# DarioSamo/sm64rt-legacy-renderer

Hardware: AMD Instinct MI355X
Metric: Mrays/s (primary+shadow), sample scene 1080p 1spp (higher is better)
Workload: dtype f32

## Files before the change

### sm64rt-legacy-renderer_amd/csrc/pass_common.h

```cpp
#pragma once
#include <type_traits>
#include "kernels.h"
#include "shade.h"

struct Pixel { uint32_t x, y; bool valid; };

enum TileShape { TILE_SQUARE = 0, TILE_ROWS = 1 };
template <int SHAPE> struct TileDim { static constexpr int W = SHAPE == TILE_SQUARE ? 16 : 32, H = SHAPE == TILE_SQUARE ? 16 : 8; };

DEV uint32_t owned_strips(PRef P) {
    const uint32_t all = (uint32_t)(P.tileY1 - P.tileY0 + 15) / 16;
    return all > (uint32_t)P.stripRank ? (all - (uint32_t)P.stripRank + (uint32_t)P.stripCount - 1) / (uint32_t)P.stripCount : 0u;
}
template <int SHAPE = TILE_SQUARE> DEV uint32_t tile_count(PRef P) {
    return (uint32_t)((P.width + TileDim<SHAPE>::W - 1) / TileDim<SHAPE>::W) * owned_strips(P) * (16u / TileDim<SHAPE>::H);
}
template <int SHAPE = TILE_SQUARE> DEV Pixel tile_pixel_at(PRef P, uint32_t tile, uint32_t wave, uint32_t lane) {
    constexpr uint32_t TW = TileDim<SHAPE>::W, TH = TileDim<SHAPE>::H, perStrip = 16u / TH;
    const uint32_t tilesX = ((uint32_t)P.width + TW - 1) / TW;
    const uint32_t tx = tile % tilesX, lt = tile / tilesX;
    const uint32_t strip = (lt / perStrip) * (uint32_t)P.stripCount + (uint32_t)P.stripRank;
    Pixel p;
    if (SHAPE == TILE_SQUARE) { p.x = tx * TW + (wave & 1) * 8 + (lane & 7); p.y = (wave >> 1) * 8 + (lane >> 3); }
    else { p.x = tx * TW + (lane & 31); p.y = wave * 2 + (lane >> 5); }
    p.y += (uint32_t)P.tileY0 + strip * 16 + (lt % perStrip) * TH;
    p.valid = p.x < (uint32_t)P.width && p.y < (uint32_t)P.tileY1;
    return p;
}
template <int SHAPE = TILE_SQUARE> DEV Pixel tile_pixel(PRef P, uint32_t tile) {
    return tile_pixel_at<SHAPE>(P, tile, threadIdx.x >> 6, threadIdx.x & 63);
}

DEV bool row_owned(PRef P, int y) { return (((y - P.tileY0) / 16) % P.stripCount) == P.stripRank; }

constexpr uint32_t stack_words(bool cached) { return cached ? RT_STACK_LDS_CACHED / 2 : RT_STACK_LDS; }
DEV TraceStack make_stack(PRef P, uint32_t *ldsStack, uint32_t wordsPerLane) {
    TraceStack s;
    uint32_t *block = ldsStack + (threadIdx.x >> 6) * wordsPerLane * RT_LANES;
    s.lds = (LdsU32Ptr)(block + (threadIdx.x & 63u));
    s.lds16 = (LdsI16Ptr)block + (threadIdx.x & 63u);
    s.spill = (GlobalU32Ptr)(P.traversalStack + ((size_t)blockIdx.x * blockDim.x + threadIdx.x) * (RT_STACK_SPILL_HEADER + RT_STACK_SPILL) + RT_STACK_SPILL_HEADER);
    s.cache = nullptr; s.ldsEntries = RT_STACK_LDS;
    return s;
}
DEV void light_columns(ShadeEnv &env, float *intensities, uint8_t *indices, uint32_t slots) {
    const uint32_t at = (threadIdx.x >> 6) * slots * RT_LANES + (threadIdx.x & 63u);
    env.lightIntensity = intensities + at; env.lightIndex = indices + at;
}

DEV uint32_t light_slots(PRef P) { return (P.lightCount < RT64_MAX_LIGHTS ? P.lightCount : (uint32_t)RT64_MAX_LIGHTS) + 1u; }


template <bool CACHED> DEV void traversal_env(PRef P, ShadeEnv &env, uint32_t *ldsStack, const u32x4_lds *dynLds) {
    env.stk = make_stack(P, ldsStack, stack_words(CACHED)); env.cnt = TraceCounts(); env.shadowRays = 0;
    env.lightIntensity = nullptr; env.lightIndex = nullptr;
    if (CACHED) env.stk.use_cache(dynLds);
}
template <bool CACHED, bool STATIC_COLUMNS = true, int BLOCK = RT_BLOCK>
DEV void shading_env(PRef P, ShadeEnv &env, uint32_t *ldsStack, float *ldsLightIntensity, uint8_t *ldsLightIndex, u32x4_lds *dynLds) {
    env.stk = make_stack(P, ldsStack, stack_words(CACHED)); env.cnt = TraceCounts(); env.shadowRays = 0;
    if (STATIC_COLUMNS) light_columns(env, ldsLightIntensity, ldsLightIndex, RT64_MAX_LIGHTS + 1);
    if (STATIC_COLUMNS && !CACHED) return;
    if (CACHED) { fill_scene_cache(P, dynLds); env.stk.use_cache(dynLds); }
    float *li = reinterpret_cast<float *>(dynLds + (CACHED ? P.cacheWords : 0u));
    light_columns(env, li, reinterpret_cast<uint8_t *>(li + light_slots(P) * (CACHED ? blockDim.x : (uint32_t)BLOCK)), light_slots(P));
}

DEV void flush_env(PRef P, const ShadeEnv &env, int pass, int rayCounter, uint32_t rays) {
    flush_counts(P, env.cnt, pass);
    if (!P.countTraversal) return;
    unsigned long long a = rays, b = env.shadowRays;
#pragma unroll
    for (int d = 32; d >= 1; d >>= 1) { a += __shfl_down(a, d, 64); b += __shfl_down(b, d, 64); }
    if ((threadIdx.x & 63) == 0) { unsigned long long *ctr = P.counters + (size_t)(blockIdx.x % RT_COUNTER_STRIPES) * CTR_COUNT; if (a) atomicAdd(&ctr[rayCounter], a); if (b) atomicAdd(&ctr[CTR_SHADOW], b); }
}

struct SurfaceHit { float key, t, u, v; uint32_t instance, prim; bool hit; };

template <bool KLIST, bool CACHED = false>
DEV uint32_t trace_surface(PRef P, ShadeEnv &env, IRef I, size_t pixel, f3 o, f3 d, const RayDiff &rayDiff,
                           uint32_t px, uint32_t py, SurfaceHit &best) {
    float oo[3] = { o.x, o.y, o.z }, dd[3] = { d.x, d.y, d.z };
    best.hit = false; best.key = INFINITY;
    uint32_t nhits = 0;
    const size_t stride = (size_t)P.width * (size_t)P.height;
    trace_ray<CACHED>(P, oo, dd, RT_RAY_MIN_DISTANCE, RT_RAY_MAX_DISTANCE, true, env.stk,
              [&](float t, float u, float v, uint32_t instance, uint32_t prim, float &tmax, uint32_t instFlags, float instDepthBias) -> bool {
                  const GpuInstance &in = P.instances[instance];
                  const float key = t - instDepthBias;
                  if (!KLIST) {
                      if (key < best.key) { best.key = key; best.t = t; best.u = u; best.v = v; best.instance = instance; best.prim = prim; best.hit = true; }
                  }
                  else {
                      if (in.cc.optTextureEdge) {
                          HitRecord tmp;
                          if (!surface_anyhit(P, instance, prim, t, u, v, d, rayDiff, px, py, tmp)) return false;
                      }
                      uint32_t hi = nhits < RT64_MAX_HIT_QUERIES ? nhits : RT64_MAX_HIT_QUERIES;
                      while (hi > 0) {
                          const uint4 prev = I.klistA[(size_t)(hi - 1) * stride + pixel];
                          if (!(key < __uint_as_float(prev.x))) break;
                          I.klistA[(size_t)hi * stride + pixel] = prev;
                          I.klistB[(size_t)hi * stride + pixel] = I.klistB[(size_t)(hi - 1) * stride + pixel];
                          hi--;
                      }
                      if (hi < RT64_MAX_HIT_QUERIES) {
                          I.klistA[(size_t)hi * stride + pixel] = make_uint4(__float_as_uint(key), __float_as_uint(u), __float_as_uint(v), prim);
                          I.klistB[(size_t)hi * stride + pixel] = make_uint2(__float_as_uint(t), instance);
                          ++nhits;
                          if (hi == RT64_MAX_HIT_QUERIES - 1 && t < tmax) tmax = t;
                      }
                      if (!(instFlags & GPU_INST_OPAQUE)) return false;
                  }
                  const float lim = key + P.maxDepthBias;
                  if (lim < tmax) tmax = lim;
                  return false;
              }, env.cnt);
    return KLIST ? nhits : (best.hit ? 1u : 0u);
}

constexpr int TRACE_WAVES = 4;
static unsigned rt_grid(const FrameParams &P) {
    const unsigned tiles = owned_tiles(P, true);
    return tiles < 1u ? 1u : (tiles < (unsigned)RT_GRID_BLOCKS ? tiles : (unsigned)RT_GRID_BLOCKS);
}
static size_t cached_lds_bytes(const FrameParams &P, bool lights) {
    const size_t slots = (P.lightCount < RT64_MAX_LIGHTS ? P.lightCount : (uint32_t)RT64_MAX_LIGHTS) + 1u;
    return (size_t)P.cacheWords * 16 + (lights ? (slots * RT_BLOCK * 5 + 15) / 16 * 16 : 0);
}
static inline dim3 image_grid(int w, int rows) { return dim3((unsigned)(w + 31) / 32, (unsigned)(rows + 7) / 8); }
template <class... Params, class... Args>
static inline void enqueue(void (*kernel)(Params...), dim3 grid, unsigned block, size_t ldsBytes, hipStream_t s, const Args &... args) {
    hipLaunchKernelGGL(kernel, grid, dim3(block), ldsBytes, s, args...);
}
template <class... Params, class... Args>
static inline hipError_t launch(void (*kernel)(Params...), dim3 grid, unsigned block, size_t ldsBytes, hipStream_t s, const Args &... args) {
    enqueue(kernel, grid, block, ldsBytes, s, args...);
    return hipGetLastError();
}
template <class F> static inline auto with_flag(bool flag, F &&f) { return flag ? f(std::true_type()) : f(std::false_type()); }
```

### sm64rt-legacy-renderer_amd/csrc/passes.hip

```cpp
#include "pass_common.h"
#include "raster_pixel.h"

#ifdef RT_ASSUME_SIMPLE
#define RT_LAUNCHER(name) name##_simple
#define RT_ROUTE_SIMPLE(call)
#else
#define RT_LAUNCHER(name) name
#define RT_ROUTE_SIMPLE(call) if (P.simpleKernels) return call
#endif

namespace {

DEV void klist_slot(PRef P, IRef I, size_t pixel, uint32_t hit, uint4 &a, uint2 &b) {
    const size_t stride = (size_t)P.width * (size_t)P.height;
    a = I.klistA[(size_t)hit * stride + pixel];
    b = I.klistB[(size_t)hit * stride + pixel];
}
template <bool KLIST>
DEV bool surface_entry(PRef P, IRef I, size_t pixel, uint32_t hit, const SurfaceHit &best, SurfaceHit &e) {
    if (!KLIST) { e = best; return true; }
    if (hit > RT64_MAX_HIT_QUERIES) return false;
    uint4 a; uint2 b; klist_slot(P, I, pixel, hit, a, b);
    e.instance = b.y; e.prim = a.w; e.t = __uint_as_float(b.x); e.u = __uint_as_float(a.y); e.v = __uint_as_float(a.z); e.hit = true; e.key = __uint_as_float(a.x);
    return true;
// ... 198 lines not shown
        f3 indirect = mk3(q_f16(P.ambientBaseColor[0] + P.ambientNoGIColor[0]), q_f16(P.ambientBaseColor[1] + P.ambientNoGIColor[1]), q_f16(P.ambientBaseColor[2] + P.ambientNoGIColor[2]));
        result = diffuse * (directStored + indirect);
        result = lerp3(diffuse, result, d.w);
    }
    else result = xyz(d);
    return result;
}
DEV void compose_lean_pixel(PRef P, IRef I, size_t i, f3 directStored) {
    f4 d = load_rgba8(I.diffuse, i);
    f3 result;
    if (d.w > RT_EPSILON) {
        f3 diffuse = xyz(d);
        f3 indirect = mk3(q_f16(P.ambientBaseColor[0] + P.ambientNoGIColor[0]), q_f16(P.ambientBaseColor[1] + P.ambientNoGIColor[1]), q_f16(P.ambientBaseColor[2] + P.ambientNoGIColor[2]));
        result = diffuse * (directStored + indirect);
        result = lerp3(diffuse, result, d.w);
    }
    else result = xyz(d);
    reinterpret_cast<float4 *>(I.output)[i] = make_float4(result.x, result.y, result.z, 1.0f);
    if (!P.separatePost) store_rgba8(I.final, i, result.x, result.y, result.z, 1.0f);
}

template <bool CACHED>
DEV f3 direct_light_pixel(PRef P, ShadeEnv &env, uint32_t px, uint32_t py, f3 rayDirection, int instanceId, f3 position, f3 normal, f3 specular) {
    f3 selfLight; float specularExponent;
    waterfall((uint32_t)instanceId, [&](uint32_t k) { const RT64_MATERIAL mk = load_const(&P.instances[k].material); selfLight = ld_v3(mk.selfLight); specularExponent = mk.specularExponent; });
    f3 resDirect = compute_lights_random<CACHED>(P, env, px, py, rayDirection, (uint32_t)instanceId, position, normal, specular, P.maxLights, true);
    resDirect = resDirect + selfLight;
    float eyeLambert = fmaxf(dot3(normal, -rayDirection), 0.0f);
    f3 eyeReflected = reflect3(rayDirection, normal);
    float eyeSpec = s_pow(fmaxf(saturatef(dot3(eyeReflected, -rayDirection)), 0.0f), specularExponent);
    f3 eyeD = mk3(P.eyeLightDiffuseColor[0], P.eyeLightDiffuseColor[1], P.eyeLightDiffuseColor[2]), eyeS = mk3(P.eyeLightSpecularColor[0], P.eyeLightSpecularColor[1], P.eyeLightSpecularColor[2]);
    return resDirect + (eyeD * eyeLambert + eyeS * (specular * eyeSpec));
}

template <bool FULL, bool CACHED = false>
__global__ __launch_bounds__(RT_BLOCK, DIRECT_WAVES) void direct_kernel(FrameParams Pv, ViewImages Iv, int cur) {
    PRef P = *kernel_params(); IRef I = *kernel_images(); (void)Pv; (void)Iv; (void)I;
    __shared__ uint32_t ldsStack[stack_words(CACHED) * RT_BLOCK];
    __shared__ float ldsLightIntensity[CACHED ? 1 : (RT64_MAX_LIGHTS + 1) * RT_BLOCK];
    __shared__ uint8_t ldsLightIndex[CACHED ? 1 : (RT64_MAX_LIGHTS + 1) * RT_BLOCK];
    extern __shared__ u32x4_lds dynLds[];
    ShadeEnv env; shading_env<CACHED>(P, env, ldsStack, ldsLightIntensity, ldsLightIndex, dynLds);
    const uint32_t tiles = tile_count<DIRECT_TILE>(P);
    for (uint32_t tile = blockIdx.x; tile < tiles; tile += gridDim.x) {
        PRef P = *kernel_params_here(); IRef I = *kernel_images_here();
        Pixel p = tile_pixel<DIRECT_TILE>(P, tile);
        if (!p.valid) continue;
        const uint32_t px = p.x, py = p.y;
        const size_t i = (size_t)py * (size_t)P.width + px;
        const int instanceId = I.instanceId[i];
        if (instanceId < 0) {
            store_rgba16f(I.directLight[cur], i, 1.0f, 1.0f, 1.0f, 0.0f);
            if (FULL) store_rgba16f(I.filteredDirect[1], i, 1.0f, 1.0f, 1.0f, 0.0f);
            else compose_lean_pixel(P, I, i, mk3s(1.0f));
            continue;
        }
        f3 o, rayDirection; f2 ndc;
        primary_ray(P, px, py, o, rayDirection, ndc);
        const float4 pos4 = reinterpret_cast<const float4 *>(I.shadingPosition)[i];
        f3 position = mk3(pos4.x, pos4.y, pos4.z), normal = xyz(load_rgba16f(I.shadingNormal, i)), specular = xyz(load_rgba16f(I.shadingSpecular, i));
        f3 newDirect = mk3s(0.0f); float historyLength = 0.0f;
        if (P.diReproject) {
            long j; float w = history_weight(P, I, i, px, py, normal, cur, j);
            f4 prevAccum = j >= 0 ? load_rgba16f(I.directLight[cur ^ 1], (size_t)j) : mk4(0, 0, 0, 0);
            newDirect = xyz(prevAccum); historyLength = prevAccum.w * w;
        }
        const f3 resDirect = direct_light_pixel<CACHED>(P, env, px, py, rayDirection, instanceId, position, normal, specular);
        historyLength = fminf(historyLength + 1.0f, 64.0f);
        newDirect = lerp3(newDirect, resDirect, s_rcp(historyLength));
        store_rgba16f(I.directLight[cur], i, newDirect.x, newDirect.y, newDirect.z, historyLength);
        if (FULL) store_rgba16f(I.filteredDirect[1], i, newDirect.x, newDirect.y, newDirect.z, historyLength);
        else compose_lean_pixel(P, I, i, mk3(q_f16(newDirect.x), q_f16(newDirect.y), q_f16(newDirect.z)));
    }
    flush_env(P, env, PASS_DIRECT, CTR_PRIMARY, 0);
}

constexpr int LEAN_WAVES = 3;
DEV bool wave_tile_of(uint32_t seq, uint32_t tiles, uint32_t &tileSeq, uint32_t &quadrant) {
    const uint32_t xcd = seq & 7u, j = seq >> 3;
    quadrant = j & 3u; tileSeq = (j >> 2) * 8u + xcd;
    return tileSeq < tiles;
}
template <bool CACHED, bool FULL, int WAVES, int BLOCK = RT_BLOCK>
__global__ __launch_bounds__(BLOCK, WAVES) void lean_frame_kernel(FrameParams Pv, ViewImages Iv, int32_t *hitInstance, int cur, int ownedY0, int ownedY1) {
    PRef P = *kernel_params(); IRef I = *kernel_images(); (void)Pv; (void)Iv; (void)I;
    __shared__ uint32_t ldsStack[stack_words(CACHED) * BLOCK];
    extern __shared__ u32x4_lds dynLds[];
    ShadeEnv env; shading_env<CACHED, false, BLOCK>(P, env, ldsStack, nullptr, nullptr, dynLds);
    uint32_t rays = 0;
    TraceCounts primaryCnt = TraceCounts();
    const uint32_t tiles = tile_count(P);
    const uint32_t trips = BLOCK == RT_BLOCK ? tiles : ((tiles + 7u) / 8u) * 32u;
    if (P.tileTiming && (threadIdx.x & 63u) == 0u) {
        uint32_t hwId; asm volatile("s_getreg_b32 %0, hwreg(HW_REG_HW_ID)" : "=s"(hwId));
        P.tileTiming[2 * ((size_t)blockIdx.x * (BLOCK / 64) + (threadIdx.x >> 6))] = make_uint4((uint32_t)__builtin_amdgcn_s_memrealtime(), (uint32_t)__builtin_amdgcn_s_memtime(), hwId, 1u);
    }
    __shared__ uint32_t ldsTripCost;
    uint32_t tileOfTrip = 0xFFFFFFFFu, visitsBefore = 0;
    const bool costed = BLOCK != RT_BLOCK && P.tileCost != nullptr;
    if (costed && threadIdx.x == 0) ldsTripCost = 0;
    auto note_cost = [&]() { if (costed) atomicMax(&ldsTripCost, env.cnt.nodes + env.cnt.tris - visitsBefore); };
    auto flush_cost = [&](PRef P) {
        if (!costed || tileOfTrip == 0xFFFFFFFFu) return;
        __syncthreads();
        if (threadIdx.x == 0) { atomicMax(&P.tileCost[tileOfTrip], ldsTripCost); ldsTripCost = 0; }
        tileOfTrip = 0xFFFFFFFFu;
    };
    for (uint32_t trip = blockIdx.x; trip < trips; trip += gridDim.x) {
        PRef P = *kernel_params_here(); IRef I = *kernel_images_here();
        Pixel p;
        if (BLOCK == RT_BLOCK) p = tile_pixel(P, tiles - 1u - trip);
        else {
            uint32_t tileSlot, quadrant;
            flush_cost(P);
            if (!wave_tile_of(trip, tiles, tileSlot, quadrant)) continue;
            tileOfTrip = P.tileOrder ? P.tileOrder[tileSlot] : tileSlot;
            p = tile_pixel_at(P, tiles - 1u - tileOfTrip, quadrant, threadIdx.x & 63u);
            visitsBefore = env.cnt.nodes + env.cnt.tris;
        }
        if (!p.valid) continue;
        const uint32_t px = p.x, py = p.y;
        const size_t i = (size_t)py * (size_t)P.width + px;
        f3 o, rayDirection; f2 ndc;
        primary_ray(P, px, py, o, rayDirection, ndc);
        RayDiff noDiff; noDiff.dOdx = noDiff.dOdy = noDiff.dDdx = noDiff.dDdy = mk3s(0.0f);
        SurfaceHit h;
        const TraceCounts before = env.cnt;
        const uint32_t nhits = trace_surface<false, CACHED>(P, env, I, i, o, rayDirection, noDiff, px, py, h);
        primaryCnt.nodes += env.cnt.nodes - before.nodes; primaryCnt.tris += env.cnt.tris - before.tris;
        rays++;
        const bool keepRecords = FULL || hitInstance != nullptr;
        if (keepRecords) {
            uint4 rec;
            if (h.hit) { rec.x = __float_as_uint(h.t); rec.y = __float_as_uint(h.u); rec.z = __float_as_uint(h.v); rec.w = h.prim; hitInstance[i] = (int32_t)h.instance; }
            else { rec.x = rec.y = rec.z = rec.w = 0xFFFFFFFFu; hitInstance[i] = -1; }
            reinterpret_cast<uint4 *>(I.primaryHit)[i] = rec;
        }

        PrimaryResolve R;
        resolve_primary<false, false, FULL>(P, I, env, px, py, i, o, rayDirection, ndc, h, nhits, R);
        if (FULL) {
            store_primary<true>(P, I, i, cur, rayDirection, R);
            if ((int)py < ownedY0 || (int)py >= ownedY1) { note_cost(); continue; }
        }
        const f4 diffuse = mk4(q_unorm8(R.color.x), q_unorm8(R.color.y), q_unorm8(R.color.z), q_unorm8(R.color.w));
        f3 direct = mk3s(1.0f); float historyLength = 0.0f;
        if (R.instanceId >= 0) {
            const f3 normal = mk3(q_f16(R.normal.x), q_f16(R.normal.y), q_f16(R.normal.z));
            const f3 specular = mk3(q_f16(R.specular.x), q_f16(R.specular.y), q_f16(R.specular.z));
            const f3 resDirect = direct_light_pixel<CACHED>(P, env, px, py, rayDirection, R.instanceId, R.position, normal, specular);
            historyLength = 1.0f;
            direct = lerp3(mk3s(0.0f), resDirect, s_rcp(historyLength));
        }
        if (keepRecords) store_rgba16f(I.directLight[cur], i, direct.x, direct.y, direct.z, historyLength);
        if (FULL) { store_rgba16f(I.filteredDirect[1], i, direct.x, direct.y, direct.z, historyLength); note_cost(); continue; }
        const f3 result = compose_lean_value(P, diffuse, mk3(q_f16(direct.x), q_f16(direct.y), q_f16(direct.z)));
        if (P.separatePost) reinterpret_cast<float4 *>(I.output)[i] = make_float4(result.x, result.y, result.z, 1.0f);
        else {
            uint32_t bits = (uint32_t)to_unorm8(result.x) | ((uint32_t)to_unorm8(result.y) << 8) | ((uint32_t)to_unorm8(result.z) << 16) | ((uint32_t)to_unorm8(1.0f) << 24);
            if (P.rasterFgCount) {
                const int wx0 = __builtin_amdgcn_readfirstlane((int)(px & ~7u)), wy0 = __builtin_amdgcn_readfirstlane((int)(py & ~7u));
                bool loaded = true, dirty = false;
                raster_blend_pixel(P.rasterFg, static_cast<const RasterTri *>(P.rasterFgTris), P.rasterFgCount, P.textures, (int)px, (int)py, true, wx0, wx0 + 7, wy0, wy0 + 7, nullptr, bits, loaded, dirty);
            }
            reinterpret_cast<uint32_t *>(I.final)[i] = bits;
            if (P.finalPacked) {
                const uint32_t rel = py - (uint32_t)P.tileY0, prow = ((rel >> 4) / (uint32_t)P.stripCount) * 16u + (rel & 15u);
                P.finalPacked[(size_t)prow * (size_t)P.width + px] = bits;
            }
        }
        note_cost();
    }
    flush_cost(P);
    if (P.tileTiming) {
        uint32_t worst = env.cnt.nodes + env.cnt.tris, total = worst;
#pragma unroll
        for (int d = 32; d >= 1; d >>= 1) { worst = max(worst, (uint32_t)__shfl_xor((int)worst, d, 64)); total += (uint32_t)__shfl_xor((int)total, d, 64); }
        if ((threadIdx.x & 63u) == 0u)
            P.tileTiming[2 * ((size_t)blockIdx.x * (BLOCK / 64) + (threadIdx.x >> 6)) + 1] = make_uint4((uint32_t)__builtin_amdgcn_s_memrealtime(), (uint32_t)__builtin_amdgcn_s_memtime(), worst, (total << 8) | 1u);
    }
    TraceCounts directCnt = TraceCounts(); directCnt.nodes = env.cnt.nodes - primaryCnt.nodes; directCnt.tris = env.cnt.tris - primaryCnt.tris;
    flush_counts(P, primaryCnt, PASS_PRIMARY_TRACE);
    env.cnt = directCnt;
    flush_env(P, env, PASS_DIRECT, CTR_PRIMARY, rays);
}


template <bool KLIST, bool CACHED>
DEV f3 second_bounce_radiance(PRef P, ShadeEnv &env, IRef I, size_t i, uint32_t px, uint32_t py, f3 rayOrigin, f3 normal, uint32_t noiseFrame, f3 ambientBase, f3 ambient) {
    const f3 rayDirection = cos_hemisphere_blue_noise(P, px, py, noiseFrame, normal);
    RayDiff rd; rd.dOdx = rd.dOdy = rd.dDdx = rd.dDdy = mk3s(0.0f);
    SurfaceHit best;
    const uint32_t nhits = trace_surface<KLIST, CACHED>(P, env, I, i, rayOrigin, rayDirection, rd, px, py, best);
    f3 resPosition = mk3s(0.0f), resNormal = mk3s(0.0f), resSpecular = mk3s(0.0f); f4 resColor = mk4(0, 0, 0, 1); int resInstanceId = -1;
    for (uint32_t hit = 0; hit < nhits; hit++) {
        HitRecord r;
        if (!surface_record<KLIST>(P, I, i, hit, best, rayDirection, rd, px, py, r)) continue;
        f4 hitColor = r.color;
        float alphaContrib = resColor.w * hitColor.w;
        if (alphaContrib >= RT_EPSILON) {
            const RT64_MATERIAL &m = P.instances[r.instanceId].material;
            resPosition = rayOrigin + rayDirection * (r.dist + m.depthBias);
            resNormal = r.normal; resSpecular = ld_v3(m.specularColor) * r.specular;
            resColor.x += hitColor.x * alphaContrib; resColor.y += hitColor.y * alphaContrib; resColor.z += hitColor.z * alphaContrib;
            resColor.w *= (1.0f - hitColor.w);
            resInstanceId = (int)r.instanceId;
        }
        if (resColor.w <= RT_EPSILON) break;
    }
    f3 resIndirect = ambientBase;
    if (resInstanceId >= 0) {
// ... 610 lines not shown
        const f3 bgColor = sky_over_background_envmap(P, rayDirection);
        RayDiff rd; rd.dOdx = rd.dOdy = rd.dDdx = rd.dDdy = mk3s(0.0f);
        SurfaceHit best;
        const uint32_t nhits = trace_surface<KLIST, CACHED>(P, env, I, i, shadingPosition, rayDirection, rd, px, py, best);
        rays++;
        const RT64_MATERIAL &pm = P.instances[instanceId].material;
        f3 resPosition = mk3s(0.0f), resNormal = mk3s(0.0f), resSpecular = mk3s(0.0f), resTransparent = mk3s(0.0f); f4 resColor = mk4(0, 0, 0, 1); int resInstanceId = -1;
        for (uint32_t hit = 0; hit < nhits; hit++) {
            HitRecord r;
            if (!surface_record<KLIST>(P, I, i, hit, best, rayDirection, rd, px, py, r)) continue;
            f4 hitColor = r.color;
            float alphaContrib = resColor.w * hitColor.w;
            if (alphaContrib >= RT_EPSILON) {
                const RT64_MATERIAL &m = P.instances[r.instanceId].material;
                bool usesLighting = m.lightGroupMaskBits > 0;
                f3 vertexPosition = shadingPosition + rayDirection * (r.dist + m.depthBias);
                if (m.fogEnabled) {
                    f4 fog = fog_from_origin(m, vertexPosition, shadingPosition);
                    resTransparent = resTransparent + xyz(fog) * (fog.w * alphaContrib);
                    alphaContrib *= (1.0f - fog.w);
                }
                f3 vertexNormal = r.normal;
                f3 specular = ld_v3(m.specularColor) * r.specular;
                if (m.reflectionFactor > RT_EPSILON) {
                    float fresnelAmount = fresnel_reflect_amount(vertexNormal, rayDirection, m.reflectionFactor, pm.reflectionFresnelFactor);
                    newReflectionAlpha += fresnelAmount * alphaContrib * reflectionAlpha;
                }
                if (usesLighting) { resColor.x += hitColor.x * alphaContrib; resColor.y += hitColor.y * alphaContrib; resColor.z += hitColor.z * alphaContrib; }
                else resTransparent = resTransparent + (xyz(hitColor) * alphaContrib) * (ambient + ld_v3(m.selfLight));
                resPosition = vertexPosition; resNormal = vertexNormal; resSpecular = specular; resInstanceId = (int)r.instanceId;
                resColor.w *= (1.0f - hitColor.w);
            }
            if (resColor.w <= RT_EPSILON) break;
        }
        f3 rgb = xyz(resColor);
        if (resInstanceId >= 0) {
            f3 directLight = compute_lights_random<CACHED>(P, env, px, py, rayDirection, (uint32_t)resInstanceId, resPosition, resNormal, resSpecular, 1, false) + ld_v3(P.instances[resInstanceId].material.selfLight);
            rgb = rgb * (ambient + directLight);
            I.reflState0[i] = make_uint4(__float_as_uint(resPosition.x), __float_as_uint(resPosition.y), __float_as_uint(resPosition.z), (uint32_t)resInstanceId);
            I.reflState1[i] = make_uint4(pack_rgba16f_lo(rayDirection.x, rayDirection.y), pack_rgba16f_lo(rayDirection.z, 0.0f), pack_rgba16f_lo(resNormal.x, resNormal.y), pack_rgba16f_lo(resNormal.z, 0.0f));
            I.reflTag[i] = frameTag;
        }
        rgb = rgb + (bgColor * resColor.w + resTransparent);
        const f3 HighlightColor = mk3(1.0f, 1.05f, 1.2f), ShadowColor = mk3(0.1f, 0.05f, 0.0f);
        float shine = pm.reflectionShineFactor;
        rgb = lerp3(rgb, HighlightColor, s_pow(fmaxf(rayDirection.y, 0.0f) * shine, 3.0f));
        rgb = lerp3(rgb, ShadowColor, s_pow(fmaxf(-rayDirection.y, 0.0f) * shine, 3.0f));
        float k = reflectionAlpha * saturatef(1.0f - newReflectionAlpha);
        store_rgba16f(I.reflection, i, refl.x + rgb.x * k, refl.y + rgb.y * k, refl.z + rgb.z * k, saturatef(newReflectionAlpha));
        if (pass < 3 && q_f16(saturatef(newReflectionAlpha)) > RT_EPSILON) I.reflectFlags[parity * 4 + pass + 1] = 1u;
    }
    flush_env(P, env, PASS_REFLECTION, CTR_REFLECTION, rays);
}

}

hipError_t RT_LAUNCHER(launch_primary_shade)(const FrameParams &P, const ViewImages &I, const int32_t *hitInstance, int cur, bool transparentLighting, bool lean, hipStream_t s) {
    RT_ROUTE_SIMPLE(launch_primary_shade_simple(P, I, hitInstance, cur, transparentLighting, lean, s));
    if (transparentLighting) return launch(primary_shade_kernel<true, true, true>, rt_grid(P), RT_BLOCK, 0, s, P, I, hitInstance, cur);
    if (lean) return launch(primary_shade_kernel<false, false, false>, rt_grid(P), RT_BLOCK, 0, s, P, I, hitInstance, cur);
    return launch(primary_shade_kernel<false, false, true>, rt_grid(P), RT_BLOCK, 0, s, P, I, hitInstance, cur);
}
hipError_t RT_LAUNCHER(launch_direct)(const FrameParams &P, const ViewImages &I, int cur, bool lean, hipStream_t s) {
    RT_ROUTE_SIMPLE(launch_direct_simple(P, I, cur, lean, s));
    return with_flag(!lean, [&](auto FULL) { return with_flag(P.cacheWords != 0, [&](auto CACHED) {
        return launch(direct_kernel<decltype(FULL)::value, decltype(CACHED)::value>, rt_grid(P), RT_BLOCK, CACHED ? cached_lds_bytes(P, true) : 0, s, P, I, cur);
    }); });
}
hipError_t RT_LAUNCHER(launch_lean_frame)(const FrameParams &P, const ViewImages &I, int32_t *hitInstance, int cur, bool full, int ownedY0, int ownedY1, unsigned maxGroups, hipStream_t s) {
    RT_ROUTE_SIMPLE(launch_lean_frame_simple(P, I, hitInstance, cur, full, ownedY0, ownedY1, maxGroups, s));
    const unsigned tiles = owned_tiles(P);
    if (maxGroups < 1u || maxGroups > RT_MAX_FRAME_GROUPS) maxGroups = RT_MAX_FRAME_GROUPS;
    unsigned grid; size_t lds = cached_lds_bytes(P, true);
    if (P.cacheWords) {
        const unsigned perGroup = (tiles + maxGroups - 1u) / maxGroups;
        grid = tiles < 1u ? 1u : (tiles + perGroup - 1u) / perGroup;
    }
    else {
        const unsigned trips = ((tiles + 7u) / 8u) * 32u, cap = maxGroups * 4u, perGroup = (trips + cap - 1u) / cap;
        grid = trips < 1u ? 32u : (trips + perGroup - 1u) / perGroup;
        grid = (grid + 31u) / 32u * 32u;
        lds = lds / (RT_BLOCK / 64) + 16;
    }
    return with_flag(P.cacheWords != 0, [&](auto CACHED) { return with_flag(full, [&](auto FULL) {
        constexpr int BLOCK = decltype(CACHED)::value ? RT_BLOCK : 64;
        return launch(lean_frame_kernel<decltype(CACHED)::value, decltype(FULL)::value, LEAN_WAVES, BLOCK>, grid, BLOCK, lds, s, P, I, hitInstance, cur, ownedY0, ownedY1);
    }); });
}
hipError_t RT_LAUNCHER(launch_indirect)(const FrameParams &P, const ViewImages &I, int cur, bool writeFiltered, bool klist, int walk, unsigned groups, int writeGuide, hipStream_t s) {
    RT_ROUTE_SIMPLE(launch_indirect_simple(P, I, cur, writeFiltered, klist, walk, groups, writeGuide, s));
    const bool second = P.giBounces >= 2u, cached = P.cacheWords != 0;
    if (klist || P.giSamples == 0 || !I.bounceRecords)
        return with_flag(klist, [&](auto KLIST) { return with_flag(second, [&](auto SECOND) {
            return launch(indirect_kernel<decltype(KLIST)::value, decltype(SECOND)::value>, rt_grid(P), RT_BLOCK, 0, s, P, I, cur, writeFiltered ? 1 : 0);
        }); });
    unsigned grid = rt_grid(P);
    {
        const unsigned tiles = owned_tiles(P), most = P.cacheWords ? RT_MAX_BOUNCE_GROUPS : RT_MAX_FRAME_GROUPS , cap = groups && groups < most ? groups : most;
        const unsigned per = tiles > cap ? (tiles + cap - 1) / cap : 1u;
        if (walk != BOUNCE_WALK_REFILL) grid = tiles < 1u ? 1u : (tiles + per - 1) / per;
    }
    if (walk == BOUNCE_WALK_REFILL) enqueue(bounce_trace_refill_kernel, grid, RT_BLOCK, 0, s, P, I);
    else with_flag(cached, [&](auto CACHED) {
        if (walk == BOUNCE_WALK_SPLIT) enqueue(bounce_trace_split_kernel<decltype(CACHED)::value>, grid, RT_BLOCK, CACHED ? cached_lds_bytes(P, false) : 0, s, P, I);
        else enqueue(bounce_trace_plain_kernel<decltype(CACHED)::value>, grid, RT_BLOCK, CACHED ? cached_lds_bytes(P, false) : 0, s, P, I);
    });
    with_flag(cached, [&](auto CACHED) { with_flag(second, [&](auto SECOND) {
        enqueue(bounce_hit_kernel<decltype(CACHED)::value, decltype(SECOND)::value>, grid, RT_BLOCK, CACHED ? cached_lds_bytes(P, true) : 0, s, P, I);
    }); });
    if (walk == BOUNCE_WALK_REFILL) enqueue(bounce_miss_kernel, grid, RT_BLOCK, 0, s, P, I);
    return launch(bounce_resolve_kernel, image_grid(P.width, P.tileY1 - P.tileY0), 256, 0, s, P, I, cur, writeFiltered ? 1 : 0, writeGuide);
}

static unsigned sparse_grid(const FrameParams &P) {
    const unsigned tiles = owned_tiles(P);
    return tiles < 1u ? 1u : (tiles < RT_MAX_FRAME_GROUPS ? tiles : RT_MAX_FRAME_GROUPS);
}
hipError_t RT_LAUNCHER(launch_refraction)(const FrameParams &P, const ViewImages &I, bool klist, hipStream_t s) {
    RT_ROUTE_SIMPLE(launch_refraction_simple(P, I, klist, s));
    return with_flag(klist, [&](auto KLIST) { return launch(refraction_kernel<decltype(KLIST)::value>, sparse_grid(P), RT_BLOCK, 0, s, P, I); });
}
hipError_t RT_LAUNCHER(launch_reflection)(const FrameParams &P, const ViewImages &I, bool klist, int pass, bool last, int parity, hipStream_t s) {
    RT_ROUTE_SIMPLE(launch_reflection_simple(P, I, klist, pass, last, parity, s));
    if (klist) return launch(reflection_kernel<true>, sparse_grid(P), RT_BLOCK, 0, s, P, I, pass, last ? 1 : 0, parity);
    if (P.cacheWords) return launch(reflection_kernel<false, true>, sparse_grid(P), RT_BLOCK, cached_lds_bytes(P, true), s, P, I, pass, last ? 1 : 0, parity);
    return launch(reflection_kernel<false>, sparse_grid(P), RT_BLOCK, 0, s, P, I, pass, last ? 1 : 0, parity);
}
```

### sm64rt-legacy-renderer_amd/csrc/rt64_gpu.h

```cpp
#pragma once
#include <stdint.h>
#include "../../include/rt64.h"

#define RT64_LEAF_BIT 0x80000000u
#define RT64_NO_CHILD 0xFFFFFFFFu
#define RT64_MAX_MIPS 16
#define RT64_MAX_LIGHTS 16
#define RT64_MAX_HIT_QUERIES 16

struct alignas(16) GpuNode {
    float lmin[3], lmax[3];
    float rmin[3], rmax[3];
    uint32_t left, right, parent, pad;
};
static_assert(sizeof(GpuNode) == 64, "GpuNode");

struct alignas(16) GpuTri {
    float v0[3]; uint32_t prim;
    float v1[3]; uint32_t pad1;
    float v2[3]; uint32_t pad2;
};
static_assert(sizeof(GpuTri) == 48, "GpuTri");
#define GPU_TRI_FETCH_SLACK_BYTES (sizeof(GpuNode) - sizeof(GpuTri))
static_assert(GPU_TRI_FETCH_SLACK_BYTES == 16 && GPU_TRI_FETCH_SLACK_BYTES <= sizeof(GpuTri), "a triangle is fetched as one node-sized record");
inline size_t gpu_tri_array_bytes(size_t triangles) { return triangles * sizeof(GpuTri) + GPU_TRI_FETCH_SLACK_BYTES; }

struct BlasHeader {
    float bmin[3]; uint32_t count;
    float bmax[3]; uint32_t depth;
};

struct GpuTexture {
    const uint8_t *texels;
    uint32_t width, height, mips, pow2;
    uint32_t mipOffset[RT64_MAX_MIPS];
};

struct GpuCombiner {
    int8_t c[2][4];
    int8_t inputCount, useTex0, useTex1, vertexUV;
    int8_t doSingle[2], doMultiply[2], doMix[2];
    int8_t colorAlphaSame, optAlpha, optTextureEdge, optNoise;
    int16_t vertexSize, normalOffset, uvOffset, inputOffset[4];
};

enum : uint32_t {
    GPU_INST_CULL_DISABLE = 1u << 0,
    GPU_INST_OPAQUE       = 1u << 1,
    GPU_INST_NORMAL_MAP   = 1u << 2,
    GPU_INST_SPECULAR_MAP = 1u << 3,
    GPU_INST_SHADOW_OPAQUE = 1u << 4,
};

struct alignas(16) GpuInstance {
    float objectToWorld[16];
    float objectToWorldNormal[16];
    float objectToWorldPrevious[16];
    float worldToObject[16];
    const GpuNode *nodes;
    const GpuTri *tris;
    const uint8_t *vertices;
    const uint32_t *indices;
    const BlasHeader *header;
    RT64_MATERIAL material;
    GpuCombiner cc;
    int32_t texDiffuse, texNormal, texSpecular;
    uint32_t filter, hAddr, vAddr;
    uint32_t flags;
    uint32_t triCount;
    uint32_t meshVersion;
    uint32_t cacheNodeOffset;
};

struct alignas(16) GpuRasterInstance {
    const uint8_t *vertices;
    const uint32_t *indices;
    uint32_t vertexStride, triCount;
    uint32_t firstTri;
    GpuCombiner cc;
    int32_t texDiffuse;
    uint32_t filter, hAddr, vAddr;
    int32_t scissorRect[4], viewportRect[4];
    uint32_t meshVersion;
    uint32_t texSerial;
};

struct FrameParams {
    float view[16], viewI[16], prevViewI[16], projection[16], projectionI[16], viewProj[16], prevViewProj[16];
    float cameraU[4], cameraV[4], cameraW[4];
    float viewport[4], resolution[4];
    float ambientBaseColor[4], ambientNoGIColor[4], eyeLightDiffuseColor[4], eyeLightSpecularColor[4];
    float skyDiffuseMultiplier[4], skyHSLModifier[4];
    float pixelJitter[2];
    float skyYawOffset, giDiffuseStrength, giSkyStrength, motionBlurStrength;
    int32_t skyPlaneTexIndex;
    uint32_t randomSeed, diSamples, giSamples, diReproject, giReproject, binaryLockMask, maxLights, motionBlurSamples;
    uint32_t visualizationMode, frameCount;
    int32_t width, height;
    int32_t tileY0, tileY1;
    int32_t stripRank, stripCount;
    float maxDepthBias;
    GpuTexture background;
    float rtViewport[4]; int32_t rtScissor[4];
    uint32_t cacheWords, cacheInstances;
    const void *cacheImage;
    uint32_t simpleKernels;
    uint32_t separatePost;
    const float *postSource; int32_t postSourceW, postSourceH;
    const GpuRasterInstance *rasterFg; const void *rasterFgTris; uint32_t rasterFgCount, rasterFgPad;
    uint32_t *finalPacked;
    float skyBase[4];
    const uint32_t *skyTiled; uint32_t skyTiledLog2W, skyTiledLog2H;
    uint32_t lightCount, instanceCount, countTraversal;
    uint32_t *tileCost; const uint32_t *tileOrder;
    uint32_t giBounces;
    const GpuInstance *instances;
    const GpuNode *tlasNodes;
    const uint32_t *tlasIndex;
    const GpuTexture *textures;
    const RT64_LIGHT *lights;
    const uint8_t *blueNoise;
    uint32_t *traversalStack;
    uint4 *tileTiming;
    unsigned long long *counters;
};

struct BounceRadiance { float r, g, b; };

struct ViewImages {
    uint16_t *viewDirection;
    float *shadingPosition;
    uint16_t *shadingNormal, *shadingSpecular;
    uint8_t *diffuse;
    int32_t *instanceId, *firstInstanceId;
    uint16_t *directLight[2], *indirectLight[2], *filteredDirect[2], *filteredIndirect[2];
    uint16_t *reflection, *refraction, *transparent;
    uint16_t *flow;
    uint8_t *reactiveMask, *lockMask;
    uint16_t *normal[2];
    float *depth[2];
    float *output;
    uint8_t *final;
    uint32_t *primaryHit;
    float *moments[2];
    uint4 *bounceRecords;
    uint32_t *bounceLists, *bounceCounts;
    BounceRadiance *bounceResults;
    uint4 *svgfGuide;
    uint32_t *svgfYoung;
    uint4 *reflState0, *reflState1; uint32_t *reflTag;
    uint32_t *reflectFlags;
    uint4 *klistA;
    uint2 *klistB;
    uint32_t *klistCount;
};

#if defined(__HIPCC__)
#define RT64_HD __host__ __device__ inline
#else
#define RT64_HD inline
#endif
#define RT64_GATHER_MAX_RANKS 64
struct GatherLayout { int height, count, mode; int starts[RT64_GATHER_MAX_RANKS + 1]; };
RT64_HD int gather_band_rows(int height, int count) { return (height + count - 1) / count; }
RT64_HD int gather_row_owner(const GatherLayout &L, int y, int *packed) {
    if (L.count <= 1) { *packed = y; return 0; }
    if (L.mode == 2) { int r = 0; while (r + 1 < L.count && y >= L.starts[r + 1]) r++; *packed = y - L.starts[r]; return r; }
    if (L.mode == 1) { const int b = gather_band_rows(L.height, L.count); *packed = y % b; return y / b; }
    const int strip = y / 16;
    *packed = (strip / L.count) * 16 + (y & 15);
    return strip % L.count;
}
RT64_HD int gather_owned_rows(const GatherLayout &L, int rank) {
    if (L.count <= 1) return L.height;
    if (L.mode == 2) return L.starts[rank + 1] - L.starts[rank];
    if (L.mode == 1) { const int b = gather_band_rows(L.height, L.count), y0 = rank * b, y1 = (rank + 1) * b; return (y1 < L.height ? y1 : L.height) - (y0 < L.height ? y0 : L.height); }
    int rows = 0;
    for (int y = rank * 16; y < L.height; y += L.count * 16) rows += (y + 16 <= L.height ? 16 : L.height - y);
    return rows;
}
RT64_HD int gather_max_owned_rows(const GatherLayout &L) {
    if (L.mode == 2) { int m = 0; for (int r = 0; r < L.count; r++) { const int n = L.starts[r + 1] - L.starts[r]; m = n > m ? n : m; } return m; }
    return L.mode == 1 ? gather_band_rows(L.height, L.count) : (((L.height + 15) / 16 + L.count - 1) / L.count) * 16;
}
RT64_HD GatherLayout gather_layout(int height, int count, int mode) { GatherLayout L; L.height = height; L.count = count < 1 ? 1 : count; L.mode = mode; for (int i = 0; i <= RT64_GATHER_MAX_RANKS; i++) L.starts[i] = 0; return L; }

#define RT_COUNTER_STRIPES 64
enum { CTR_NODES = 0, CTR_TRIS, CTR_PRIMARY, CTR_SHADOW, CTR_INDIRECT, CTR_REFLECTION, CTR_REFRACTION,
       CTR_PASS_BASE,
       CTR_COUNT = CTR_PASS_BASE + 2 * 6 };
enum { PASS_PRIMARY_TRACE = 0, PASS_PRIMARY_SHADE, PASS_DIRECT, PASS_INDIRECT, PASS_REFRACTION, PASS_REFLECTION };
```

### sm64rt-legacy-renderer_amd/csrc/rt64_host.cpp

```cpp
#include <algorithm>
#include <chrono>
#include <cmath>
#include <cstdio>
#include <cstdlib>
#include <cstring>
#include <map>
#include <stdexcept>
#include <string>
#include <vector>

#include "kernels.h"
#include "device_math.h"

#define RT64_EXPORT extern "C" __attribute__((visibility("default")))

namespace rt64 {

static std::string GlobalLastError;

#define HIP_CHECK(call) do { hipError_t e_ = (call); if (e_ != hipSuccess) { \
    char msg_[512]; snprintf(msg_, sizeof(msg_), "HIP call " #call " failed: %s", hipGetErrorString(e_)); throw std::runtime_error(msg_); } } while (0)

template <class T> struct DevArray {
    T *ptr = nullptr; size_t count = 0;
// ... 20 lines not shown
static Mat4 mat_transpose(const Mat4 &A) { Mat4 R; for (int i = 0; i < 4; i++) for (int j = 0; j < 4; j++) R.m[i * 4 + j] = A.m[j * 4 + i]; return R; }

static Mat4 mat_inverse(const Mat4 &M) {
    double m[16], inv[16];
    for (int i = 0; i < 16; i++) m[i] = (double)M.m[i];
    inv[0] = m[5] * m[10] * m[15] - m[5] * m[11] * m[14] - m[9] * m[6] * m[15] + m[9] * m[7] * m[14] + m[13] * m[6] * m[11] - m[13] * m[7] * m[10];
    inv[4] = -m[4] * m[10] * m[15] + m[4] * m[11] * m[14] + m[8] * m[6] * m[15] - m[8] * m[7] * m[14] - m[12] * m[6] * m[11] + m[12] * m[7] * m[10];
    inv[8] = m[4] * m[9] * m[15] - m[4] * m[11] * m[13] - m[8] * m[5] * m[15] + m[8] * m[7] * m[13] + m[12] * m[5] * m[11] - m[12] * m[7] * m[9];
    inv[12] = -m[4] * m[9] * m[14] + m[4] * m[10] * m[13] + m[8] * m[5] * m[14] - m[8] * m[6] * m[13] - m[12] * m[5] * m[10] + m[12] * m[6] * m[9];
    inv[1] = -m[1] * m[10] * m[15] + m[1] * m[11] * m[14] + m[9] * m[2] * m[15] - m[9] * m[3] * m[14] - m[13] * m[2] * m[11] + m[13] * m[3] * m[10];
    inv[5] = m[0] * m[10] * m[15] - m[0] * m[11] * m[14] - m[8] * m[2] * m[15] + m[8] * m[3] * m[14] + m[12] * m[2] * m[11] - m[12] * m[3] * m[10];
    inv[9] = -m[0] * m[9] * m[15] + m[0] * m[11] * m[13] + m[8] * m[1] * m[15] - m[8] * m[3] * m[13] - m[12] * m[1] * m[11] + m[12] * m[3] * m[9];
    inv[13] = m[0] * m[9] * m[14] - m[0] * m[10] * m[13] - m[8] * m[1] * m[14] + m[8] * m[2] * m[13] + m[12] * m[1] * m[10] - m[12] * m[2] * m[9];
    inv[2] = m[1] * m[6] * m[15] - m[1] * m[7] * m[14] - m[5] * m[2] * m[15] + m[5] * m[3] * m[14] + m[13] * m[2] * m[7] - m[13] * m[3] * m[6];
    inv[6] = -m[0] * m[6] * m[15] + m[0] * m[7] * m[14] + m[4] * m[2] * m[15] - m[4] * m[3] * m[14] - m[12] * m[2] * m[7] + m[12] * m[3] * m[6];
    inv[10] = m[0] * m[5] * m[15] - m[0] * m[7] * m[13] - m[4] * m[1] * m[15] + m[4] * m[3] * m[13] + m[12] * m[1] * m[7] - m[12] * m[3] * m[5];
    inv[14] = -m[0] * m[5] * m[14] + m[0] * m[6] * m[13] + m[4] * m[1] * m[14] - m[4] * m[2] * m[13] - m[12] * m[1] * m[6] + m[12] * m[2] * m[5];
    inv[3] = -m[1] * m[6] * m[11] + m[1] * m[7] * m[10] + m[5] * m[2] * m[11] - m[5] * m[3] * m[10] - m[9] * m[2] * m[7] + m[9] * m[3] * m[6];
    inv[7] = m[0] * m[6] * m[11] - m[0] * m[7] * m[10] - m[4] * m[2] * m[11] + m[4] * m[3] * m[10] + m[8] * m[2] * m[7] - m[8] * m[3] * m[6];
    inv[11] = -m[0] * m[5] * m[11] + m[0] * m[7] * m[9] + m[4] * m[1] * m[11] - m[4] * m[3] * m[9] - m[8] * m[1] * m[7] + m[8] * m[3] * m[5];
    inv[15] = m[0] * m[5] * m[10] - m[0] * m[6] * m[9] - m[4] * m[1] * m[10] + m[4] * m[2] * m[9] + m[8] * m[1] * m[6] - m[8] * m[2] * m[5];
    double det = m[0] * inv[0] + m[1] * inv[4] + m[2] * inv[8] + m[3] * inv[12];
    Mat4 R = {};
    if (det == 0.0) return R;
    double r = 1.0 / det;
    for (int i = 0; i < 16; i++) R.m[i] = (float)(inv[i] * r);
    return R;
}

static Mat4 mat_perspective_fov_rh(float fov, float aspect, float zn, float zf) {
    float s = sinf(0.5f * fov), c = cosf(0.5f * fov);
    float h = c / s, w = h / aspect, range = zf / (zn - zf);
    Mat4 P = {};
    P.m[0] = w; P.m[5] = h; P.m[10] = range; P.m[11] = -1.0f; P.m[14] = range * zn;
    return P;
}

struct V3 { float x, y, z; };
static V3 v3(float x, float y, float z) { V3 r = { x, y, z }; return r; }
static V3 operator+(V3 a, V3 b) { return v3(a.x + b.x, a.y + b.y, a.z + b.z); }
static V3 operator-(V3 a, V3 b) { return v3(a.x - b.x, a.y - b.y, a.z - b.z); }
static V3 operator*(V3 a, float s) { return v3(a.x * s, a.y * s, a.z * s); }
static float vlen(V3 a) { return sqrtf(a.x * a.x + a.y * a.y + a.z * a.z); }
static V3 vnorm(V3 a) { float l = vlen(a); return l > 0.0f ? v3(a.x / l, a.y / l, a.z / l) : a; }
static V3 vcross(V3 a, V3 b) { return v3(a.y * b.z - a.z * b.y, a.z * b.x - a.x * b.z, a.x * b.y - a.y * b.x); }
static V3 mat_point(const Mat4 &M, V3 p) { return v3(p.x * M.m[0] + p.y * M.m[4] + p.z * M.m[8] + 1.0f * M.m[12], p.x * M.m[1] + p.y * M.m[5] + p.z * M.m[9] + 1.0f * M.m[13], p.x * M.m[2] + p.y * M.m[6] + p.z * M.m[10] + 1.0f * M.m[14]); }
static V3 mat_vector(const Mat4 &M, V3 p) { return v3(p.x * M.m[0] + p.y * M.m[4] + p.z * M.m[8] + 0.0f * M.m[12], p.x * M.m[1] + p.y * M.m[5] + p.z * M.m[9] + 0.0f * M.m[13], p.x * M.m[2] + p.y * M.m[6] + p.z * M.m[10] + 0.0f * M.m[14]); }


static GpuCombiner decode_combiner(uint32_t shaderId) {
    GpuCombiner cc = {};
    for (int i = 0; i < 4; i++) { cc.c[0][i] = (int8_t)((shaderId >> (i * 3)) & 7); cc.c[1][i] = (int8_t)((shaderId >> (12 + i * 3)) & 7); }
    for (int i = 0; i < 2; i++) for (int j = 0; j < 4; j++) {
        int v = cc.c[i][j];
        if (v >= 1 && v <= 4 && v > cc.inputCount) cc.inputCount = (int8_t)v;
        if (v == 5 || v == 6) cc.useTex0 = 1;
        if (v == 7) cc.useTex1 = 1;
    }
    for (int i = 0; i < 2; i++) {
        cc.doSingle[i] = cc.c[i][2] == 0;
        cc.doMultiply[i] = cc.c[i][1] == 0 && cc.c[i][3] == 0;
        cc.doMix[i] = cc.c[i][1] == cc.c[i][3];
    }
    cc.colorAlphaSame = (shaderId & 0xfff) == ((shaderId >> 12) & 0xfff);
    cc.optAlpha = (shaderId & (1u << 24)) != 0;
    cc.optTextureEdge = (shaderId & (1u << 26)) != 0;
    cc.optNoise = (shaderId & (1u << 27)) != 0;
    cc.vertexUV = cc.useTex0 || cc.useTex1;
    int sz = 16;
    cc.normalOffset = (int16_t)sz; sz += 12;
    cc.uvOffset = (int16_t)sz; if (cc.vertexUV) sz += 8;
    for (int i = 0; i < cc.inputCount; i++) { cc.inputOffset[i] = (int16_t)sz; sz += cc.optAlpha ? 16 : 12; }
    cc.vertexSize = (int16_t)sz;
    return cc;
}


#define RT64_RENDER_STREAMS_MAX 4
#define RT64_LEAN_HOLDOFF_FRAMES 4

struct Options {
    bool countTraversal = false, profilePasses = true, syncPresent = true, alwaysRebuild = false, leanFrames = true, fusedLean = true, foldForeground = true;
    int profileEvery = 1;
    bool leanRecords = false;
    bool framePrologue = true;
    bool hostTlas = true;
    bool simpleKernels = true;
    bool ldsCache = true;
    bool tileTiming = false;
    int bounceGroups = -1;
    int bounceSplit = -1;
    int bounceRefill = -1;
    int denoiserMode = 1;
    bool tileOrder = true;
    bool foldCompose = true;
    bool foldVariance = true;
    bool foldGuide = true;
    bool overlapFrames = true;
    bool overlapReflection = true;
    bool haloExchange = false;
    bool haloDryRun = false;
    int haloMargin = SVGF_INPUT_HALO_ROWS;
    int maxReflections = 2;
    uint32_t motionBlurSamples = 32;
    int visualizationMode = 0;
    bool generateMipmaps = false;
    int giBounces = 1;
    int primarySpp = 1;
    unsigned maxFrameGroups = RT_MAX_FRAME_GROUPS;
};

struct Device {
    int hipDevice = 0;
    hipStream_t stream = nullptr;
    hipStream_t streams[RT64_RENDER_STREAMS_MAX] = {}; int cur = 0, streamCount = 3;
    hipEvent_t streamJoin[RT64_RENDER_STREAMS_MAX] = {};
    bool streamBusy[RT64_RENDER_STREAMS_MAX] = {};
    bool framePure = false, lastFramePure = false;
    void joinStreams() {
        for (int k = 0; k < streamCount; k++) {
            if (k == cur || !streamBusy[k]) continue;
            HIP_CHECK(hipEventRecord(streamJoin[k], streams[k]));
            HIP_CHECK(hipStreamWaitEvent(stream, streamJoin[k], 0));
            streamBusy[k] = false;
        }
    }
    unsigned long long orderedEpoch = 1, seenEpoch[RT64_RENDER_STREAMS_MAX] = {};
    hipEvent_t streamCatchUp = nullptr;
    void noteOrderedWork() { seenEpoch[cur] = ++orderedEpoch; }
    void impure() { framePure = false; joinStreams(); noteOrderedWork(); }
    void enter() { use(); joinStreams(); noteOrderedWork(); lastFramePure = false; }
    void switchStream() {
        const int prev = cur;
        streamBusy[prev] = true; cur = (cur + 1) % streamCount; stream = streams[cur];
        if (seenEpoch[cur] != orderedEpoch) {
            HIP_CHECK(hipEventRecord(streamCatchUp, streams[prev]));
            HIP_CHECK(hipStreamWaitEvent(stream, streamCatchUp, 0));
            seenEpoch[cur] = orderedEpoch;
        }
    }
    int width = 0, height = 0, pendingWidth = 0, pendingHeight = 0;
    int tileY0 = 0, tileY1 = 0; bool tileSet = false;
    int stripRank = 0, stripCount = 1;
    struct DrawnPartition { int tileY0 = 0, tileY1 = 0, stripRank = 0, stripCount = 1; bool valid = false; } drawn;
    std::vector<Scene *> scenes;
    Options opt;
    RT64_FRAME_STATS stats = {}, accum = {}; bool statsPending = false, statsHaveView = false;
    bool profNow = false, statsProfiled = false; unsigned profCounter = 0;
    double hostUpdateUs = 0.0, hostRenderUs = 0.0, hostStageUs[16] = {}, hostEventUs = 0.0; unsigned long long hostFrames = 0;
    void finishStats();
    uint32_t *traversalOverflow = nullptr;
    void checkTraversalOverflow();
    DevArray<uint32_t> spillStack[RT64_RENDER_STREAMS_MAX];
    DevArray<uint32_t> querySlab; uint32_t *queryOverflow = nullptr; hipEvent_t querySlabDone = nullptr, queryOrder = nullptr; bool querySlabUsed = false;
    DevArray<uint8_t> queryRays, queryHits, querySurfaces, queryLods, queryMaterials, queryVisibility, queryLighting, queryPixels, queryDiffs, queryFootprints;
    DevArray<uint8_t> queryBounces, queryReflected, queryRefracted;
    void awaitQueries();
    void *gatherTarget = nullptr; size_t gatherTargetBytes = 0;
    hipEvent_t frameWait = nullptr;
    uint8_t *finalOverride = nullptr;
    hipStream_t auxStream = nullptr; hipEvent_t forkEvent = nullptr, joinEvent = nullptr;
    struct HaloLink {
        RT64_HALO_EXCHANGE fn = nullptr; void *user = nullptr; int rank = 0, count = 0; std::vector<int> starts;
        struct Gather *gather = nullptr;
        hipEvent_t ready = nullptr, done = nullptr;
        uint8_t *pinned = nullptr; size_t pinnedBytes = 0;
// ... 79 lines not shown
    uint32_t blasCount = 0;
    float hostBmin[3] = { 0, 0, 0 }, hostBmax[3] = { 0, 0, 0 };
    uint32_t topologyVersion = 0, depth = 255;
    uint32_t treeDepth() const { return blasCount == 0 ? 0u : depth; }
    bool buildPending = false, pendingRefit = false;
    ~Mesh();
    uint32_t version = 0;
    std::map<int, std::pair<float, float>> alphaBounds; uint32_t alphaBoundsVersion = 0;
    Mesh(Device *d, int f) : device(d), flags(f) {}
    void set(const void *vertexArray, int vcount, int vstride, const unsigned int *indexArray, int icount);
    std::pair<float, float> inputAlphaBounds(int offset);
};

struct Instance {
    Scene *scene;
    Mesh *mesh = nullptr; Texture *diffuse = nullptr, *normal = nullptr, *specular = nullptr; Shader *shader = nullptr;
    Mat4 transform = mat_identity(), previousTransform = mat_identity();
    RT64_MATERIAL material = {}; RT64_RECT scissorRect = {}, viewportRect = {}; unsigned int flags = 0;
    explicit Instance(Scene *s);
    ~Instance();
};

struct Scene {
    Device *device; RT64_SCENE_DESC desc = {};
    std::vector<RT64_LIGHT> lights;
    std::vector<Instance *> instances; std::vector<View *> views;
    explicit Scene(Device *d);
    ~Scene();
};

struct RenderInstance { Instance *instance; };

struct View {
    Scene *scene;
    float resolutionScale = 1.0f, motionBlurStrength = 0.0f; uint32_t diSamples = 0, giSamples = 0, maxLights = 12;
    bool denoiserEnabled = false;
    int upscaler = RT64_UPSCALER_OFF, upscalerMode = RT64_UPSCALER_MODE_AUTO; float upscalerSharpness = 0.0f;
    bool upscaleActive = false; int jitterPhases = 1; float pixelJitter[2] = { 0.0f, 0.0f };
    float *upscaled[2] = { nullptr, nullptr }; int upW = 0, upH = 0, upSwap = 0; bool upValid = false;
    float *sharpened = nullptr; int sharpW = 0, sharpH = 0; bool sharpValid = false;
    bool sharpenActive() const { return upscaleActive && upscalerSharpness > 0.0f; }
    void releaseSharpened() { if (sharpened) hipFree(sharpened); sharpened = nullptr; sharpW = sharpH = 0; sharpValid = false; }
    Texture *skyPlane = nullptr;
    DevArray<uint32_t> skyTiled; uint32_t skyTiledSerial = 0; uint32_t skyTiledLog2[2] = { 0, 0 };
    Mat4 view = mat_identity(), projection = mat_identity(), viewI = mat_identity(), projectionI = mat_identity(), viewProj = mat_identity(), prevViewI = mat_identity(), prevViewProj = mat_identity();
    float fov = 0.0f, nearDist = 0.0f, farDist = 0.0f; bool canReproject = true, matricesValid = false, perspectiveSet = false;
    uint32_t frameCount = 0; bool rtSwap = false, skipReprojection = true;
    int imgW = 0, imgH = 0;
    int finalW = 0, finalH = 0;
    float rtViewport[4] = { 0, 0, 0, 0 }; int rtScissor[4] = { 0, 0, 0, 0 }; bool rtRect = false;
    bool needSpillSlab = false;
    uint32_t cacheWords = 0;
    bool separatePost() const { return upscaleActive || rtRect || imgW != finalW || imgH != finalH || (motionBlurStrength > 0.0f && scene->device->opt.motionBlurSamples > 0); }
    ViewImages img = {};
    std::vector<void *> allocations; uint32_t bounceSamples = 0;
    DevArray<int32_t> hitInstance;
    std::vector<RenderInstance> rtInstances, rasterBg, rasterFg;
    struct RasterList {
        DevArray<GpuRasterInstance> table; DevArray<uint8_t> tris;
        std::vector<uint8_t> uploaded;
        uint32_t triTotal = 0; int w = 0, h = 0, y0 = 0, y1 = 0; bool apply = false, ready = false, changed = false;
        bool contentChanged = false;
        int bounds[4] = { 0, 0, 0, 0 };
    };
    RasterList rasterBgEnv, rasterBgScreen, rasterFgScreen;
    DevArray<uint8_t> background; int backgroundW = 0, backgroundH = 0;
    void prepareRasterList(const std::vector<RenderInstance> &list, RasterList &rl, int w, int h, int y0, int y1, bool apply);
    void drawRasterList(RasterList &rl, uint8_t *target, bool clear = false);
    RasterPrologue prologue = {}; size_t prologueCopyBytes = 0;
    void flushTableCopy();
    void flushPrologue();
    void discardPrologue();
    void discardUpdate();
    std::vector<Texture *> usedTextures;
    template <class T> struct TablePtr { T *ptr = nullptr; };
    enum { TABLE_SLOTS = 2 * RT64_RENDER_STREAMS_MAX };
    struct TableSlot {
        DevArray<uint8_t> dTables; TablePtr<GpuInstance> dInstances; TablePtr<GpuTexture> dTextures; TablePtr<RT64_LIGHT> dLights;
        DevArray<GpuNode> tlasNodes; DevArray<uint32_t> tlasIndex, tlasMorton, tlasLeafParent; DevArray<BlasHeader> tlasHeader; DevArray<uint8_t> tlasScratch;
        const GpuNode *tlasNodesAt = nullptr; const uint32_t *tlasIndexAt = nullptr, *tlasMortonAt = nullptr; const BlasHeader *tlasHeaderAt = nullptr;
        std::vector<uint8_t> uploadedTables;
        DevArray<uint8_t> cacheImage; bool cacheImageValid = false;
        const uint8_t *cacheImageAt = nullptr; std::vector<uint64_t> cacheBlasKey;
        unsigned readers = 0;
        std::vector<hipEvent_t> queryEvents;
    } tab[TABLE_SLOTS];
    int tabCur = 0;
    std::vector<uint8_t> tableScratch;
    float maxDepthBias = 0.0f;
    bool anyNonOpaque = false, anyReflection = false, anyRefraction = false, anyFog = false;
    bool simpleFrame = false;
    bool leanFrame = false;
    bool fusedFullFrame = false;
    bool packedFinal = false;
    bool fusedStoreless = false;
    bool fusedFrame = false;
    FrameParams lastParams; int lastCur = 0;
    struct QueryScene {
        bool valid = false;
        bool meshDestroyed = false;
        bool textureDestroyed = false;
        FrameParams P;
        int slot = 0; bool needSpill = false;
        std::vector<std::pair<Mesh *, uint32_t>> meshes;
        std::vector<Instance *> instances;
        std::vector<std::pair<Texture *, uint32_t>> textures;
    } query;
    void snapshotQueryScene();
    void pruneQueryEvents(bool wait);
    bool reflStatePending = false; uint32_t reflStateTag = 0; int reflStateY0 = 0, reflStateY1 = 0;
    void applyReflectionState();
    int subFrame = 0, subFrames = 1; DevArray<float> sppSum;
    DevArray<uint32_t> tileCost[RT64_RENDER_STREAMS_MAX], tileOrder[RT64_RENDER_STREAMS_MAX]; uint32_t tileOrderTiles = 0; bool tileOrderValid[RT64_RENDER_STREAMS_MAX] = {};
    uint8_t *finalBuf[RT64_RENDER_STREAMS_MAX] = {};

    explicit View(Scene *s);
    ~View();
    void releaseImages();
    void createImages(int w, int h, int screenW, int screenH);
    void update();
    void render();
    void fillParams(FrameParams &P);
    void materialise();
};


static std::string assets_dir() {
    if (const char *e = getenv("RT64_ASSETS_DIR")) return e;
    Dl_info info;
    if (dladdr(reinterpret_cast<const void *>(&assets_dir), &info) && info.dli_fname) {
        std::string p = info.dli_fname;
        size_t s = p.find_last_of('/');
        if (s != std::string::npos) return p.substr(0, s) + "/../assets";
    }
    return "assets";
}

Device::Device(int w, int h, int dev) {
    int count = 0;
    hipError_t e = hipGetDeviceCount(&count);
    if (e != hipSuccess || count == 0) throw std::runtime_error("No HIP device available: librt64.so needs an AMD GPU (there is no CPU fallback).");
    if (dev < 0) { HIP_CHECK(hipGetDevice(&dev)); }
    if (dev >= count) throw std::runtime_error("Requested HIP device index is out of range.");
    hipDevice = dev;
    use();
    hipDeviceProp_t prop;
    HIP_CHECK(hipGetDeviceProperties(&prop, dev));
    if (w <= 0 || h <= 0) throw std::runtime_error("Invalid device size.");
    width = pendingWidth = w; height = pendingHeight = h; tileY0 = 0; tileY1 = h;
    if (const char *e = getenv("RT64_RENDER_STREAMS")) streamCount = std::min(std::max(atoi(e), 1), RT64_RENDER_STREAMS_MAX);
    for (int k = 0; k < streamCount; k++) {
        HIP_CHECK(hipStreamCreateWithFlags(&streams[k], hipStreamNonBlocking));
        HIP_CHECK(hipEventCreateWithFlags(&streamJoin[k], hipEventDisableTiming));
    }
    HIP_CHECK(hipEventCreateWithFlags(&streamCatchUp, hipEventDisableTiming));
    HIP_CHECK(hipHostMalloc(reinterpret_cast<void **>(&traversalOverflow), 64, hipHostMallocMapped)); *traversalOverflow = 0;
    HIP_CHECK(hipHostMalloc(reinterpret_cast<void **>(&queryOverflow), 64, hipHostMallocMapped)); *queryOverflow = 0;
    HIP_CHECK(hipEventCreateWithFlags(&querySlabDone, hipEventDisableTiming));
    HIP_CHECK(hipEventCreateWithFlags(&queryOrder, hipEventDisableTiming));
    stream = streams[0]; cur = 0; seenEpoch[0] = orderedEpoch;
    for (auto &set : eventSets) for (auto &ev : set) HIP_CHECK(hipEventCreate(&ev));
    for (auto &set : auxEvents) for (auto &ev : set) HIP_CHECK(hipEventCreate(&ev));
    counters.reserve((size_t)CTR_COUNT * RT_COUNTER_STRIPES);
    HIP_CHECK(hipMemsetAsync(counters.ptr, 0, counters.bytes(), stream));
    blueNoise.reserve(512 * 512 * 4);
    std::string path = assets_dir() + "/bluenoise_512x512_rgba8.bin";
    std::vector<uint8_t> bn(512 * 512 * 4, 128);
    if (FILE *f = fopen(path.c_str(), "rb")) {
        size_t got = fread(bn.data(), 1, bn.size(), f);
        fclose(f);
        if (got != bn.size()) throw std::runtime_error("Blue-noise table " + path + " is truncated.");
    }
    else throw std::runtime_error("Blue-noise table " + path + " not found (the library looks in <its directory>/../assets; RT64_ASSETS_DIR overrides): soft shadows and GI sampling need it.");
    HIP_CHECK(hipMemcpy(blueNoise.ptr, bn.data(), bn.size(), hipMemcpyHostToDevice));
    HIP_CHECK(hipStreamSynchronize(stream));
}

Device::~Device() {
    hipSetDevice(hipDevice);
    for (hipStream_t st : streams) if (st) hipStreamSynchronize(st);
// ... 427 lines not shown
        g.texSerial = inst->diffuse->serial;
        g.scissorRect[0] = inst->scissorRect.x; g.scissorRect[1] = inst->scissorRect.y; g.scissorRect[2] = inst->scissorRect.w; g.scissorRect[3] = inst->scissorRect.h;
        g.viewportRect[0] = inst->viewportRect.x; g.viewportRect[1] = inst->viewportRect.y; g.viewportRect[2] = inst->viewportRect.w; g.viewportRect[3] = inst->viewportRect.h;
        g.meshVersion = inst->mesh->version;
        if (g.cc.vertexSize > inst->mesh->vertexStride || inst->mesh->vertexStride < 16) throw std::runtime_error("Raster instance mesh vertex stride is smaller than the layout its shader reads.");
        triTotal += g.triCount;
        float vpX = 0.0f, vpY = 0.0f, vpW = (float)w, vpH = (float)h;
        if (apply && inst->viewportRect.w > 0 && inst->viewportRect.h > 0) { vpX = (float)inst->viewportRect.x; vpY = (float)(h - inst->viewportRect.y - inst->viewportRect.h); vpW = (float)inst->viewportRect.w; vpH = (float)inst->viewportRect.h; }
        for (int v = 0; v < inst->mesh->vertexCount; v++) {
            float p[4]; memcpy(p, inst->mesh->hostVertices.data() + (size_t)v * inst->mesh->vertexStride, 16);
            if (!(p[3] > 1e-3f) || !(fabsf(p[0]) <= 4.0f * p[3]) || !(fabsf(p[1]) <= 4.0f * p[3])) { bx0 = by0 = -1e9f; bx1 = by1 = 1e9f; continue; }
            const float rw = 1.0f / p[3], xs = ((p[0] * rw) * 0.5f + 0.5f) * vpW + vpX, ys = (0.5f - (p[1] * rw) * 0.5f) * vpH + vpY;
            bx0 = std::min(bx0, xs); bx1 = std::max(bx1, xs); by0 = std::min(by0, ys); by1 = std::max(by1, ys);
        }
    }
    const size_t bytes = hst.size() * sizeof(GpuRasterInstance);
    const bool sameContent = rl.ready && rl.uploaded.size() == bytes && memcmp(rl.uploaded.data(), hst.data(), bytes) == 0 &&
                             rl.w == w && rl.h == h && rl.y0 == y0 && rl.y1 == y1 && rl.apply == apply;
    if (sameContent && !dev->opt.alwaysRebuild) return;
    dev->impure();
    rl.contentChanged = !sameContent;
    rl.table.reserve(hst.size()); rl.tris.reserve(std::max<size_t>(raster_tri_bytes(triTotal), 16));
    const bool inlineTable = raster_setup_takes_table_inline((uint32_t)hst.size());
    if (!inlineTable) {
        uint8_t *stage = static_cast<uint8_t *>(dev->ringAlloc(bytes));
        memcpy(stage, hst.data(), bytes);
        HIP_CHECK(hipMemcpyAsync(rl.table.ptr, stage, bytes, hipMemcpyHostToDevice, dev->stream));
    }
    rl.uploaded.assign(reinterpret_cast<uint8_t *>(hst.data()), reinterpret_cast<uint8_t *>(hst.data()) + bytes);
    rl.triTotal = triTotal; rl.w = w; rl.h = h; rl.y0 = y0; rl.y1 = y1; rl.apply = apply; rl.ready = true; rl.changed = true;
    rl.bounds[0] = std::max(0, (int)std::floor(std::min(bx0, 1e9f)) - 1); rl.bounds[1] = std::max(y0, (int)std::floor(std::min(by0, 1e9f)) - 1);
    rl.bounds[2] = std::min(w, (int)std::ceil(std::max(bx1, -1e9f)) + 2); rl.bounds[3] = std::min(y1, (int)std::ceil(std::max(by1, -1e9f)) + 2);
    if (inlineTable && dev->opt.framePrologue && hst.size() <= RASTER_PROLOGUE_INSTANCES && prologue.listCount < RASTER_PROLOGUE_LISTS) {
        RasterPrologueList &L = prologue.list[prologue.listCount++];
        memset(&L, 0, sizeof(L));
        memcpy(L.inst, hst.data(), bytes);
        L.deviceTable = rl.table.ptr; L.tris = rl.tris.ptr; L.instanceCount = (uint32_t)hst.size(); L.triTotal = triTotal; L.w = w; L.h = h; L.y0 = y0; L.y1 = y1; L.apply = apply ? 1 : 0;
    }
    else if (inlineTable) HIP_CHECK(launch_raster_setup_inline(hst.data(), rl.table.ptr, (uint32_t)hst.size(), triTotal, rl.tris.ptr, w, h, y0, y1, apply, dev->stream));
    else HIP_CHECK(launch_raster_setup(rl.table.ptr, (uint32_t)hst.size(), triTotal, rl.tris.ptr, w, h, y0, y1, apply, dev->stream));
}

void View::flushTableCopy() {
    if (!prologueCopyBytes) return;
    HIP_CHECK(hipMemcpyAsync(prologue.copyDst, prologue.copySrc, prologueCopyBytes, hipMemcpyHostToDevice, scene->device->stream));
    prologueCopyBytes = 0; prologue.copySrc = nullptr; prologue.copyDst = nullptr;
}
void View::flushPrologue() {
    Device *dev = scene->device;
    if (prologue.listCount == 0) { flushTableCopy(); return; }
    prologue.copyWords = (uint32_t)((prologueCopyBytes + 15) / 16);
    if (prologueCopyBytes > (size_t)RASTER_PROLOGUE_COPY_WORDS * 16) { flushTableCopy(); prologue.copyWords = 0; }
    HIP_CHECK(launch_frame_prologue(prologue, dev->stream));
    prologueCopyBytes = 0;
    memset(&prologue, 0, sizeof(prologue));
    dev->workSinceMark = true;
}

void View::discardPrologue() {
    if (prologueCopyBytes) { tab[tabCur].uploadedTables.clear(); tab[tabCur].cacheBlasKey.clear(); tab[tabCur].cacheImageValid = false; }
    for (uint32_t i = 0; i < prologue.listCount; i++)
        for (RasterList *rl : { &rasterBgEnv, &rasterBgScreen, &rasterFgScreen })
            if (rl->table.ptr == prologue.list[i].deviceTable) { rl->ready = false; rl->uploaded.clear(); }
    memset(&prologue, 0, sizeof(prologue)); prologueCopyBytes = 0;
}
void View::discardUpdate() {
    query.valid = false;
    for (Texture *t : usedTextures) t->currentIndex = -1;
    usedTextures.clear();
    discardPrologue();
}

void View::drawRasterList(RasterList &rl, uint8_t *target, bool clear) {
    if (!rl.ready || rl.triTotal == 0) return;
    Device *dev = scene->device;
    HIP_CHECK(launch_raster_draw(rl.table.ptr, rl.tris.ptr, rl.triTotal, tab[tabCur].dTextures.ptr, target, rl.w, rl.y0, rl.y1, rl.bounds, dev->stripRank, dev->stripCount, clear, dev->stream));
    dev->workSinceMark = true;
}

#define RT64_HOST_TLAS_MAX 64
static inline float gmin(float a, float b) { return (a < b || (a == b && std::signbit(a))) ? a : b; }
static inline float gmax(float a, float b) { return (a > b || (a == b && !std::signbit(a))) ? a : b; }
static void host_build_tlas(const GpuInstance *inst, const float (*meshMin)[3], const float (*meshMax)[3], uint32_t n,
                            GpuNode *nodes, uint32_t *sortedIndex, uint32_t *morton, BlasHeader *header) {
    std::vector<float> lo(3 * (size_t)n), hi(3 * (size_t)n);
    float smin[3] = { INFINITY, INFINITY, INFINITY }, smax[3] = { -INFINITY, -INFINITY, -INFINITY };
    for (uint32_t i = 0; i < n; i++) {
        float bmn[3] = { INFINITY, INFINITY, INFINITY }, bmx[3] = { -INFINITY, -INFINITY, -INFINITY };
        for (int c = 0; c < 8; c++) {
            const float p[3] = { (c & 1) ? meshMax[i][0] : meshMin[i][0], (c & 2) ? meshMax[i][1] : meshMin[i][1], (c & 4) ? meshMax[i][2] : meshMin[i][2] };
            float w[3]; g_xform_point(inst[i].objectToWorld, p, w);
            for (int k = 0; k < 3; k++) { bmn[k] = gmin(bmn[k], w[k]); bmx[k] = gmax(bmx[k], w[k]); }
        }
        for (int k = 0; k < 3; k++) { lo[3 * i + k] = bmn[k]; hi[3 * i + k] = bmx[k]; smin[k] = gmin(smin[k], bmn[k]); smax[k] = gmax(smax[k], bmx[k]); }
    }
    std::vector<unsigned long long> keys(n);
    for (uint32_t i = 0; i < n; i++) {
        uint32_t q[3];
        for (int k = 0; k < 3; k++) {
            const float ext = smax[k] - smin[k], scale = ext > 0.0f ? 1024.0f / ext : 0.0f;
            const float c = (lo[3 * i + k] + hi[3 * i + k]) * 0.5f, f = (c - smin[k]) * scale;
            const int qi = (int)f;
            q[k] = (uint32_t)(qi < 0 ? 0 : (qi > 1023 ? 1023 : qi));
        }
        keys[i] = ((unsigned long long)host_morton30(q[0], q[1], q[2]) << 32) | i;
    }
    std::sort(keys.begin(), keys.end());
    for (uint32_t s = 0; s < n; s++) { sortedIndex[s] = (uint32_t)(keys[s] & 0xFFFFFFFFull); morton[s] = (uint32_t)(keys[s] >> 32); }
    memset(nodes, 0, sizeof(GpuNode) * std::max<uint32_t>(n - 1, 1));
    auto leafLo = [&](uint32_t s) { return &lo[3 * (size_t)sortedIndex[s]]; };
    auto leafHi = [&](uint32_t s) { return &hi[3 * (size_t)sortedIndex[s]]; };
    if (n == 1) {
        GpuNode &nd = nodes[0];
        nd.left = RT64_LEAF_BIT; nd.right = RT64_NO_CHILD; nd.parent = RT64_NO_CHILD;
        for (int k = 0; k < 3; k++) { nd.lmin[k] = leafLo(0)[k]; nd.lmax[k] = leafHi(0)[k]; nd.rmin[k] = INFINITY; nd.rmax[k] = -INFINITY; header->bmin[k] = nd.lmin[k]; header->bmax[k] = nd.lmax[k]; }
        header->count = 1; header->depth = 1;
        return;
    }
    const int N = (int)n;
    auto delta = [&](int i, int j) -> int { return (j < 0 || j >= N) ? -1 : __builtin_clzll(keys[(size_t)i] ^ keys[(size_t)j]); };
    nodes[0].parent = RT64_NO_CHILD;
    for (int i = 0; i < N - 1; i++) {
        const int d = (delta(i, i + 1) - delta(i, i - 1)) >= 0 ? 1 : -1, dmin = delta(i, i - d);
        int lmax = 2;
        while (delta(i, i + lmax * d) > dmin) lmax *= 2;
        int l = 0;
        for (int t = lmax / 2; t >= 1; t /= 2) if (delta(i, i + (l + t) * d) > dmin) l += t;
        const int j = i + l * d, dnode = delta(i, j);
        int s = 0;
        for (int div = 2;; div *= 2) { const int t = (l + div - 1) / div; if (delta(i, i + (s + t) * d) > dnode) s += t; if (t <= 1) break; }
        const int g = i + s * d + (d < 0 ? -1 : 0), lo_ = i < j ? i : j, hi_ = i < j ? j : i;
        if (lo_ == g) nodes[i].left = RT64_LEAF_BIT | (uint32_t)g; else { nodes[i].left = (uint32_t)g; nodes[g].parent = (uint32_t)i; }
        if (hi_ == g + 1) nodes[i].right = RT64_LEAF_BIT | (uint32_t)(g + 1); else { nodes[i].right = (uint32_t)(g + 1); nodes[g + 1].parent = (uint32_t)i; }
        nodes[i].pad = (uint32_t)j;
    }
    struct Fit { static uint32_t run(GpuNode *nodes, uint32_t i, const std::vector<float> &lo, const std::vector<float> &hi, const uint32_t *sorted, float *mn, float *mx) {
        GpuNode &nd = nodes[i]; uint32_t depth = 0;
        for (int side = 0; side < 2; side++) {
            const uint32_t c = side ? nd.right : nd.left;
            float *cmn = side ? nd.rmin : nd.lmin, *cmx = side ? nd.rmax : nd.lmax;
            if (c & RT64_LEAF_BIT) { const size_t inst = sorted[c & 0x7FFFFFFFu]; for (int k = 0; k < 3; k++) { cmn[k] = lo[3 * inst + k]; cmx[k] = hi[3 * inst + k]; } }
            else depth = std::max(depth, run(nodes, c, lo, hi, sorted, cmn, cmx));
        }
        for (int k = 0; k < 3; k++) { mn[k] = gmin(nd.lmin[k], nd.rmin[k]); mx[k] = gmax(nd.lmax[k], nd.rmax[k]); }
        return depth + 1;
    } };
    float rmn[3], rmx[3];
    header->depth = Fit::run(nodes, 0, lo, hi, sortedIndex, rmn, rmx);
    for (int k = 0; k < 3; k++) { header->bmin[k] = rmn[k]; header->bmax[k] = rmx[k]; }
    header->count = n;
}

void View::update() {
    Device *dev = scene->device;
    discardPrologue();
    {
        const float scale = resolutionScale > 0.0f ? resolutionScale : 1.0f;
        int rw = std::max(1, (int)lroundf((float)dev->width * scale)), rh = std::max(1, (int)lroundf((float)dev->height * scale));
        int uw = 0, uh = 0, phases = 1;
        upscaleActive = upscaler_info(upscaler, upscalerMode, dev->width, dev->height, uw, uh, phases);
        if (upscaleActive) { rw = uw; rh = uh; jitterPhases = phases; }
        if (imgW != rw || imgH != rh || finalW != dev->width || finalH != dev->height) createImages(rw, rh, dev->width, dev->height);
        if (upscaleActive && (upW != dev->width || upH != dev->height)) {
            for (auto &u : upscaled) { if (u) hipFree(u); u = nullptr; HIP_CHECK(hipMalloc(reinterpret_cast<void **>(&u), (size_t)dev->width * dev->height * 16)); }
            upW = dev->width; upH = dev->height; upValid = false;
        }
        if (!upscaleActive) upValid = false;
        if (!sharpenActive()) { if (sharpened) releaseSharpened(); }
// ... 35 lines not shown
        throw std::runtime_error("RT64_DrawDevice: resolutionScale != 1, motion blur and a viewport / scissor on the ray-traced picture resample across rows; they need the whole frame on one device (no RT64_SetDeviceTile / RT64_SetDeviceInterleave).");
    if (usedTextures.size() > 512) throw std::runtime_error("More than 512 textures in one frame (SRV_TEXTURES_MAX).");

    const size_t nInst = rtInstances.size(), nTex = usedTextures.size(), nLights = scene->lights.size();
    const size_t instBytes = nInst * sizeof(GpuInstance), texBytes = nTex * sizeof(GpuTexture), lightBytes = nLights * sizeof(RT64_LIGHT);
    tableScratch.resize(instBytes + texBytes + lightBytes + 64);
    uint8_t *stage = tableScratch.data();
    GpuInstance *hInst = reinterpret_cast<GpuInstance *>(stage);
    GpuTexture *hTex = reinterpret_cast<GpuTexture *>(stage + instBytes);
    RT64_LIGHT *hLights = reinterpret_cast<RT64_LIGHT *>(stage + instBytes + texBytes);
    std::vector<uint32_t> cacheOffset(nInst, 0);
    cacheWords = 0;
    if (dev->opt.ldsCache && nInst >= 1 && nInst <= 16) {
        uint64_t words = 4 * nInst + 4 * std::max<size_t>(nInst - 1, 1);
        for (size_t i = 0; i < nInst; i++) { cacheOffset[i] = (uint32_t)words; words += 4ull * std::max<uint32_t>(rtInstances[i].instance->mesh->blasCount - 1, 1); }
        uint32_t deepest = 0;
        if (words <= RT_CACHE_MAX_WORDS) for (size_t i = 0; i < nInst; i++) deepest = std::max(deepest, rtInstances[i].instance->mesh->treeDepth());
        if (words <= RT_CACHE_MAX_WORDS && std::max<size_t>(nInst - 1, 1) + deepest <= RT_STACK_LDS_CACHED) cacheWords = (uint32_t)words;
    }
    {
        uint32_t deepest = 0;
        for (size_t i = 0; i < nInst; i++) deepest = std::max(deepest, rtInstances[i].instance->mesh->treeDepth());
        needSpillSlab = nInst > 0 && std::max<size_t>(nInst - 1, 1) + deepest > RT_STACK_LDS;
    }
    maxDepthBias = nInst ? -INFINITY : 0.0f;
    anyNonOpaque = anyReflection = anyRefraction = anyFog = false;
    simpleFrame = dev->opt.simpleKernels && nInst > 0;
    for (size_t i = 0; i < nInst; i++) {
        Instance *inst = rtInstances[i].instance;
        GpuInstance &g = hInst[i];
        memset(&g, 0, sizeof(g));
        memcpy(g.objectToWorld, inst->transform.m, 64);
        memcpy(g.objectToWorldPrevious, subFrame > 0 ? inst->transform.m : inst->previousTransform.m, 64);
        Mat4 upper = inst->transform;
        upper.m[3] = upper.m[7] = upper.m[11] = 0.0f; upper.m[12] = upper.m[13] = upper.m[14] = 0.0f; upper.m[15] = 1.0f;
        Mat4 nrm = mat_transpose(mat_inverse(upper));
        memcpy(g.objectToWorldNormal, nrm.m, 64);
        Mat4 w2o = mat_inverse(inst->transform);
        memcpy(g.worldToObject, w2o.m, 64);
        Mesh *mesh = inst->mesh;
        g.nodes = mesh->nodes.ptr; g.tris = mesh->tris.ptr; g.vertices = mesh->vertices.ptr; g.indices = mesh->indices.ptr; g.header = mesh->header.ptr;
        g.material = inst->material;
        g.cc = inst->shader->cc;
        g.texDiffuse = g.material.diffuseTexIndex = inst->diffuse->currentIndex;
        g.texNormal = g.material.normalTexIndex = inst->normal ? inst->normal->currentIndex : -1;
        g.texSpecular = g.material.specularTexIndex = inst->specular ? inst->specular->currentIndex : -1;
        g.filter = inst->shader->filter; g.hAddr = inst->shader->hAddr; g.vAddr = inst->shader->vAddr;
        g.flags = 0;
        if (inst->flags & RT64_INSTANCE_DISABLE_BACKFACE_CULLING) g.flags |= GPU_INST_CULL_DISABLE;
        if (instance_is_opaque(inst, g.cc)) g.flags |= GPU_INST_OPAQUE;
        if (inst->shader->flags & RT64_SHADER_NORMAL_MAP_ENABLED) g.flags |= GPU_INST_NORMAL_MAP;
        if (inst->shader->flags & RT64_SHADER_SPECULAR_MAP_ENABLED) g.flags |= GPU_INST_SPECULAR_MAP;
        if (instance_is_shadow_opaque(inst, g.cc)) g.flags |= GPU_INST_SHADOW_OPAQUE;
        else simpleFrame = false;
        g.triCount = mesh->blasCount;
        g.meshVersion = mesh->version;
        g.cacheNodeOffset = cacheWords ? cacheOffset[i] : 0u;
        if (g.cc.vertexSize > mesh->vertexStride) throw std::runtime_error("Instance mesh vertex stride is smaller than the layout its shader reads.");
        maxDepthBias = std::max(maxDepthBias, inst->material.depthBias);
        if (!(g.flags & GPU_INST_OPAQUE)) anyNonOpaque = true;
        if (inst->material.reflectionFactor > 1e-6f) anyReflection = true;
        if (inst->material.refractionFactor > 1e-6f) anyRefraction = true;
        if (inst->material.fogEnabled) anyFog = true;
    }
    for (size_t i = 0; i < nTex; i++) {
        Texture *t = usedTextures[i];
        GpuTexture &g = hTex[i];
        g.texels = t->texels.ptr; g.width = (uint32_t)t->width; g.height = (uint32_t)t->height; g.mips = (uint32_t)t->mips;
        g.pow2 = ((t->width & (t->width - 1)) == 0 && (t->height & (t->height - 1)) == 0) ? 1u : 0u;
        if (!g.pow2) simpleFrame = false;
        memcpy(g.mipOffset, t->mipOffset, sizeof(g.mipOffset));
    }
    if (nLights) memcpy(hLights, scene->lights.data(), lightBytes);
    const size_t tableBytes = instBytes + texBytes + lightBytes;
    const bool sameContent = tab[tabCur].uploadedTables.size() == tableBytes && tableBytes && memcmp(tab[tabCur].uploadedTables.data(), stage, tableBytes) == 0;
    const bool unchanged = sameContent && !dev->opt.alwaysRebuild;
    if (!unchanged) {
        int pick = -1;
        pruneQueryEvents(false);
        for (int k = 1; k < TABLE_SLOTS && pick < 0; k++) { const int c = (tabCur + k) % TABLE_SLOTS; if (!(tab[c].readers & ~(1u << dev->cur)) && tab[c].queryEvents.empty()) pick = c; }
        if (pick < 0) { pick = (tabCur + 1) % TABLE_SLOTS; dev->impure(); }
        tabCur = pick;
        tab[tabCur].readers = 0;
        for (hipEvent_t ev : tab[tabCur].queryEvents) HIP_CHECK(hipStreamWaitEvent(dev->stream, ev, 0));
        const uint32_t n = (uint32_t)nInst;
        const bool hostTlas = n >= 1 && n <= RT64_HOST_TLAS_MAX && dev->opt.hostTlas;
        const size_t tlasAt = (tableBytes + 63) & ~(size_t)63, nodeBytes = sizeof(GpuNode) * std::max<size_t>(n ? n - 1 : 0, 1);
        const bool hostCache = hostTlas && cacheWords != 0;
        const size_t cacheAt = (tlasAt + nodeBytes + sizeof(BlasHeader) + 2 * sizeof(uint32_t) * n + 63) & ~(size_t)63, headWords = hostCache ? 4 * (size_t)n + 4 * std::max<size_t>(n - 1, 1) : 0;
        const size_t uploadBytes = hostTlas ? (hostCache ? cacheAt + headWords * 16 : tlasAt + nodeBytes + sizeof(BlasHeader) + 2 * sizeof(uint32_t) * n) : tableBytes;
        {
            const size_t need = (std::max<size_t>(hostCache ? cacheAt + (size_t)cacheWords * 16 : uploadBytes, 4096) + 15) & ~(size_t)15;
            if (need > tab[tabCur].dTables.count || (n && !hostTlas)) dev->impure();
            tab[tabCur].dTables.reserve(need);
        }
        tab[tabCur].dInstances.ptr = reinterpret_cast<GpuInstance *>(tab[tabCur].dTables.ptr); tab[tabCur].dTextures.ptr = reinterpret_cast<GpuTexture *>(tab[tabCur].dTables.ptr + instBytes);
        tab[tabCur].dLights.ptr = reinterpret_cast<RT64_LIGHT *>(tab[tabCur].dTables.ptr + instBytes + texBytes);
        if (uploadBytes) {
            uint8_t *pinnedStage = static_cast<uint8_t *>(dev->ringAlloc(uploadBytes));
            memcpy(pinnedStage, stage, tableBytes);
            if (hostTlas) {
                memset(pinnedStage + tableBytes, 0, tlasAt - tableBytes);
                GpuNode *hn = reinterpret_cast<GpuNode *>(pinnedStage + tlasAt);
                BlasHeader *hh = reinterpret_cast<BlasHeader *>(pinnedStage + tlasAt + nodeBytes);
                uint32_t *hi = reinterpret_cast<uint32_t *>(hh + 1), *hm = hi + n;
                float mn[RT64_HOST_TLAS_MAX][3], mx[RT64_HOST_TLAS_MAX][3];
                for (uint32_t i = 0; i < n; i++) { memcpy(mn[i], rtInstances[i].instance->mesh->hostBmin, 12); memcpy(mx[i], rtInstances[i].instance->mesh->hostBmax, 12); }
                host_build_tlas(hInst, mn, mx, n, hn, hi, hm, hh);
                if (hostCache) {
                    memset(pinnedStage + tlasAt + nodeBytes + sizeof(BlasHeader) + 2 * sizeof(uint32_t) * n, 0, cacheAt - (tlasAt + nodeBytes + sizeof(BlasHeader) + 2 * sizeof(uint32_t) * n));
                    uint32_t *cw = reinterpret_cast<uint32_t *>(pinnedStage + cacheAt);
                    for (uint32_t k = 0; k < n; k++) {
                        const uint32_t inst = hi[k]; const GpuInstance &g = hInst[inst]; const float *M = g.worldToObject;
                        for (int c = 0; c < 3; c++) { const float row[4] = { M[c], M[4 + c], M[8 + c], M[12 + c] }; memcpy(cw + 16 * k + 4 * c, row, 16); }
                        const uint64_t tp = reinterpret_cast<uint64_t>(g.tris);
                        uint32_t info[4] = { inst | ((g.flags & 0xFFu) << 8) | (g.cacheNodeOffset << 16), 0u, (uint32_t)tp, (uint32_t)(tp >> 32) };
                        memcpy(&info[1], &g.material.depthBias, 4);
                        memcpy(cw + 16 * k + 12, info, 16);
                    }
                    auto childRef = [](uint32_t c) { return (c & RT64_LEAF_BIT) ? (c == RT64_NO_CHILD ? c : (0xFFFF8000u | (c & 0x7FFFu))) : c; };
                    const uint32_t tn = std::max<uint32_t>(n - 1, 1);
                    for (uint32_t t = 0; t < tn; t++) {
                        uint32_t *dst = cw + 16 * (size_t)n + 16 * (size_t)t;
                        memcpy(dst, &hn[t], 64);
                        dst[12] = childRef(hn[t].left); dst[13] = childRef(hn[t].right);
                    }
                }
                uint8_t *base = tab[tabCur].dTables.ptr + tlasAt;
                tab[tabCur].tlasNodesAt = reinterpret_cast<const GpuNode *>(base); tab[tabCur].tlasHeaderAt = reinterpret_cast<const BlasHeader *>(base + nodeBytes);
                tab[tabCur].tlasIndexAt = reinterpret_cast<const uint32_t *>(tab[tabCur].tlasHeaderAt + 1); tab[tabCur].tlasMortonAt = tab[tabCur].tlasIndexAt + n;
            }
            prologue.copySrc = pinnedStage; prologue.copyDst = tab[tabCur].dTables.ptr; prologueCopyBytes = uploadBytes;
        }
        if (n && !hostTlas) {
            flushTableCopy();
            tab[tabCur].tlasNodes.reserve(std::max<size_t>(n - 1, 1)); tab[tabCur].tlasIndex.reserve(n); tab[tabCur].tlasMorton.reserve(n); tab[tabCur].tlasLeafParent.reserve(n); tab[tabCur].tlasHeader.reserve(1);
            LbvhArgs a = {};
            a.mode = LBVH_MODE_INSTANCES; a.refit = 0; a.n = n; a.instances = tab[tabCur].dInstances.ptr;
            a.nodes = tab[tabCur].tlasNodes.ptr; a.tris = nullptr; a.header = tab[tabCur].tlasHeader.ptr; a.sortedIndex = tab[tabCur].tlasIndex.ptr; a.morton = tab[tabCur].tlasMorton.ptr; a.leafParent = tab[tabCur].tlasLeafParent.ptr;
            if (n > LBVH_SMALL_MAX) { tab[tabCur].tlasScratch.reserve(lbvh_large_scratch_bytes(n)); a.scratch = tab[tabCur].tlasScratch.ptr; a.scratchBytes = tab[tabCur].tlasScratch.bytes(); }
            HIP_CHECK(lbvh_launch(a, dev->stream));
            tab[tabCur].tlasNodesAt = tab[tabCur].tlasNodes.ptr; tab[tabCur].tlasIndexAt = tab[tabCur].tlasIndex.ptr; tab[tabCur].tlasMortonAt = tab[tabCur].tlasMorton.ptr; tab[tabCur].tlasHeaderAt = tab[tabCur].tlasHeader.ptr;
        }
        tab[tabCur].cacheImageValid = false;
        if (hostCache) {
            tab[tabCur].cacheImageAt = tab[tabCur].dTables.ptr + cacheAt;
            std::vector<uint64_t> key; key.reserve(2 + 4 * (size_t)n);
            key.push_back(reinterpret_cast<uint64_t>(tab[tabCur].cacheImageAt)); key.push_back(cacheWords);
            for (uint32_t i = 0; i < n; i++) { key.push_back(reinterpret_cast<uint64_t>(hInst[i].nodes)); key.push_back(hInst[i].meshVersion); key.push_back(hInst[i].cacheNodeOffset); key.push_back(hInst[i].triCount); }
            if (key != tab[tabCur].cacheBlasKey) {
                flushTableCopy();
                HIP_CHECK(launch_scene_cache_image(tab[tabCur].dInstances.ptr, tab[tabCur].tlasIndexAt, tab[tabCur].tlasNodesAt, n, const_cast<uint8_t *>(tab[tabCur].cacheImageAt), true, dev->stream));
                tab[tabCur].cacheBlasKey.swap(key);
            }
            tab[tabCur].cacheImageValid = true;
        }
        else tab[tabCur].cacheBlasKey.clear();
        tab[tabCur].uploadedTables.assign(stage, stage + tableBytes);
        dev->workSinceMark = true;
    }
    if (cacheWords && !tab[tabCur].cacheImageValid) {
        dev->impure();
        flushTableCopy();
        tab[tabCur].cacheImage.reserve((size_t)cacheWords * 16);
        HIP_CHECK(launch_scene_cache_image(tab[tabCur].dInstances.ptr, tab[tabCur].tlasIndexAt, tab[tabCur].tlasNodesAt, (uint32_t)nInst, tab[tabCur].cacheImage.ptr, false, dev->stream));
        tab[tabCur].cacheImageAt = tab[tabCur].cacheImage.ptr; tab[tabCur].cacheImageValid = true;
    }
    {
        const bool whole = separatePost();
        const int sy0 = whole ? 0 : dev->tileY0, sy1 = whole ? finalH : dev->tileY1;
        prepareRasterList(rasterBg, rasterBgEnv, finalW, finalH, 0, finalH, false);
        prepareRasterList((rtInstances.empty() || rtRect || dev->opt.visualizationMode != 0) ? rasterBg : std::vector<RenderInstance>(), rasterBgScreen, finalW, finalH, sy0, sy1, true);
        prepareRasterList(rasterFg, rasterFgScreen, finalW, finalH, sy0, sy1, true);
        flushPrologue();
        if (!rasterBg.empty() && (backgroundW != finalW || backgroundH != finalH)) { background.reserve((size_t)finalW * finalH * 4); backgroundW = finalW; backgroundH = finalH; rasterBgEnv.changed = true; }
        if (leanFrame && (rasterBgEnv.contentChanged || (!rasterBgEnv.ready && lastParams.background.texels))) { materialise(); dev->leanHoldoff = RT64_LEAN_HOLDOFF_FRAMES; }
        if (rasterBgEnv.ready && rasterBgEnv.changed) {
            dev->impure();
            const bool clearInDraw = dev->opt.framePrologue && rasterBgEnv.triTotal != 0;
            if (!clearInDraw) HIP_CHECK(hipMemsetAsync(background.ptr, 0, (size_t)finalW * finalH * 4, dev->stream));
            const int sr = dev->stripRank, sc = dev->stripCount; dev->stripRank = 0; dev->stripCount = 1;
            drawRasterList(rasterBgEnv, background.ptr, clearInDraw);
            dev->stripRank = sr; dev->stripCount = sc;
        }
    }
    for (Texture *t : usedTextures) t->currentIndex = -1;
    usedTextures.clear();
}

void View::fillParams(FrameParams &P) {
    Device *dev = scene->device;
    memset(&P, 0, sizeof(P));
    const RT64_SCENE_DESC &d = scene->desc;
    auto set4 = [](float *dst, RT64_VECTOR3 v) { dst[0] = v.x; dst[1] = v.y; dst[2] = v.z; dst[3] = 0.0f; };
    set4(P.ambientBaseColor, d.ambientBaseColor); set4(P.ambientNoGIColor, d.ambientNoGIColor);
    set4(P.eyeLightDiffuseColor, d.eyeLightDiffuseColor); set4(P.eyeLightSpecularColor, d.eyeLightSpecularColor);
    set4(P.skyDiffuseMultiplier, d.skyDiffuseMultiplier); set4(P.skyHSLModifier, d.skyHSLModifier);
    P.skyYawOffset = d.skyYawOffset; P.giDiffuseStrength = d.giDiffuseStrength; P.giSkyStrength = d.giSkyStrength;

    projection = mat_perspective_fov_rh(fov, dev->aspect(), nearDist, farDist);
    const bool reproject = canReproject && matricesValid;
    if (reproject) { prevViewI = viewI; prevViewProj = viewProj; }
    viewI = mat_inverse(view); projectionI = mat_inverse(projection); viewProj = mat_mul(view, projection);
    if (!reproject) { prevViewI = viewI; prevViewProj = viewProj; }
    matricesValid = true;
    memcpy(P.view, view.m, 64); memcpy(P.viewI, viewI.m, 64); memcpy(P.prevViewI, prevViewI.m, 64); memcpy(P.projection, projection.m, 64);
    memcpy(P.projectionI, projectionI.m, 64); memcpy(P.viewProj, viewProj.m, 64); memcpy(P.prevViewProj, prevViewProj.m, 64);

    const float focal = (nearDist + farDist) / 2.0f, aspect = dev->aspect();
    V3 pos = mat_point(viewI, v3(0, 0, 0));
    V3 dir = mat_vector(viewI, v3(0, 0, 1)); { float l = vlen(dir); dir = v3(dir.x / l, dir.y / l, dir.z / l); }
    V3 target = pos + dir * focal;
    V3 W = vnorm(target - pos) * focal;
    V3 U = vnorm(vcross(W, v3(0, 1, 0)));
    V3 V = vnorm(vcross(U, W));
    const float ulen = focal * tanf(fov * 0.5f) * aspect, vlen_ = focal * tanf(fov * 0.5f);
    U = U * ulen; V = V * vlen_;
    P.cameraU[0] = U.x; P.cameraU[1] = U.y; P.cameraU[2] = U.z; P.cameraV[0] = V.x; P.cameraV[1] = V.y; P.cameraV[2] = V.z; P.cameraW[0] = W.x; P.cameraW[1] = W.y; P.cameraW[2] = W.z;
    for (int k = 0; k < 4; k++) { P.viewport[k] = rtViewport[k]; P.rtViewport[k] = rtViewport[k]; P.rtScissor[k] = rtScissor[k]; }
    P.resolution[0] = (float)imgW; P.resolution[1] = (float)imgH; P.resolution[2] = (float)dev->width; P.resolution[3] = (float)dev->height;
    pixelJitter[0] = pixelJitter[1] = 0.0f;
    if (upscaleActive) { const int fi = (int)(frameCount % (uint32_t)jitterPhases) + 1; pixelJitter[0] = halton_sequence(fi, 2) - 0.5f; pixelJitter[1] = halton_sequence(fi, 3) - 0.5f; }
    if (subFrames > 1) { pixelJitter[0] = halton_sequence(subFrame + 1, 2) - 0.5f; pixelJitter[1] = halton_sequence(subFrame + 1, 3) - 0.5f; }
    P.pixelJitter[0] = pixelJitter[0]; P.pixelJitter[1] = pixelJitter[1];
    P.motionBlurStrength = motionBlurStrength; P.motionBlurSamples = dev->opt.motionBlurSamples;
    P.skyPlaneTexIndex = skyPlane ? 0 : -1;
    P.skyTiled = nullptr; P.skyTiledLog2W = P.skyTiledLog2H = 0;
    if (skyPlane && (giSamples > 0 || anyReflection) && skyPlane->width >= 4 && skyPlane->height >= 4 &&
        (skyPlane->width & (skyPlane->width - 1)) == 0 && (skyPlane->height & (skyPlane->height - 1)) == 0) {
        if (skyTiledSerial != skyPlane->serial) {
            dev->impure();
            skyTiled.reserve((size_t)skyPlane->width * skyPlane->height);
            HIP_CHECK(tile_texture_launch(skyPlane->texels.ptr, skyTiled.ptr, (uint32_t)skyPlane->width, (uint32_t)skyPlane->height, dev->stream));
            skyTiledSerial = skyPlane->serial;
            skyTiledLog2[0] = (uint32_t)__builtin_ctz((unsigned)skyPlane->width); skyTiledLog2[1] = (uint32_t)__builtin_ctz((unsigned)skyPlane->height);
        }
        P.skyTiled = skyTiled.ptr; P.skyTiledLog2W = skyTiledLog2[0]; P.skyTiledLog2H = skyTiledLog2[1];
    }
    P.randomSeed = frameCount; P.frameCount = frameCount;
    P.diSamples = diSamples; P.giSamples = giSamples; P.maxLights = maxLights; P.giBounces = (uint32_t)dev->opt.giBounces;
    P.diReproject = 0;
    P.giReproject = (!skipReprojection && denoiserEnabled && giSamples > 0) ? 1u : 0u;
    P.binaryLockMask = upscaleActive ? 0u : 1u;
    P.visualizationMode = 0;
    P.width = imgW; P.height = imgH; P.tileY0 = dev->tileY0; P.tileY1 = dev->tileY1; P.stripRank = dev->stripRank; P.stripCount = dev->stripCount;
    P.cacheWords = cacheWords; P.cacheInstances = cacheWords ? (uint32_t)rtInstances.size() : 0u; P.cacheImage = cacheWords ? tab[tabCur].cacheImageAt : nullptr;
    P.separatePost = separatePost() ? 1u : 0u;
    P.simpleKernels = simpleFrame ? 1u : 0u;
    P.postSource = img.output; P.postSourceW = imgW; P.postSourceH = imgH;
    P.rasterFg = nullptr; P.rasterFgTris = nullptr; P.rasterFgCount = 0; P.rasterFgPad = 0; P.finalPacked = nullptr;
    memset(&P.background, 0, sizeof(P.background));
    if (rasterBgEnv.ready) { P.background.texels = background.ptr; P.background.width = (uint32_t)backgroundW; P.background.height = (uint32_t)backgroundH; P.background.mips = 1; P.background.pow2 = ((backgroundW & (backgroundW - 1)) == 0 && (backgroundH & (backgroundH - 1)) == 0) ? 1u : 0u; }
    if (P.separatePost) { P.tileY0 = 0; P.tileY1 = imgH; P.stripRank = 0; P.stripCount = 1; }
    P.maxDepthBias = maxDepthBias;
    {
        const float SCREEN_WIDTH = 320.0f, SCREEN_HEIGHT = 240.0f, SKYBOX_WIDTH = 4.0f * SCREEN_WIDTH, SKYBOX_HEIGHT = 4.0f * SCREEN_HEIGHT, PI = 3.14159265f, TWO_PI = PI * 2.0f;
        V3 vd = mat_vector(viewI, v3(0, 0, 1)); { float inv = 1.0f / vlen(vd); vd = v3(vd.x * inv, vd.y * inv, vd.z * inv); }
        auto hfmod = [](float x, float y) { return x - y * truncf(x / y); };
        float skyYawRadians = hfmod(d.skyYawOffset + atan2f(vd.x, -vd.z) + PI, TWO_PI);
        float baseX = SCREEN_WIDTH * 360.0f * (skyYawRadians - PI) / (90.0f * PI * 2.0f);
        float skyPitchRadians = atan2f(-vd.y, sqrtf(vd.x * vd.x + vd.z * vd.z));
        float pitchInDegrees = skyPitchRadians * 360.0f / (PI * 2.0f);
        float degreesToScale = 360.0f * pitchInDegrees / 90.0f;
        float baseY = degreesToScale + 5.0f * (SCREEN_HEIGHT / 2.0f);
        baseY = std::min(std::max(baseY, SCREEN_HEIGHT), SKYBOX_HEIGHT);
        float aspectRatio = P.viewport[2] / P.viewport[3];
        baseX += SCREEN_WIDTH / 2.0f;
        baseX -= (SCREEN_HEIGHT * aspectRatio) / 2.0f;
        baseX /= SKYBOX_WIDTH;
        baseY = (SKYBOX_HEIGHT - baseY) / SKYBOX_HEIGHT;
        float ratioDivision = aspectRatio / (4.0f / 3.0f);
        P.skyBase[0] = baseX; P.skyBase[1] = baseY; P.skyBase[2] = 0.25f * ratioDivision; P.skyBase[3] = 0.25f;
    }
    P.lightCount = (uint32_t)scene->lights.size(); P.instanceCount = (uint32_t)rtInstances.size();
    P.countTraversal = dev->opt.countTraversal ? 1u : 0u;
    { TableSlot &T = tab[tabCur]; P.instances = T.dInstances.ptr; P.tlasNodes = T.tlasNodesAt; P.tlasIndex = T.tlasIndexAt; P.textures = T.dTextures.ptr; P.lights = T.dLights.ptr; T.readers |= 1u << dev->cur; }
    {
        DevArray<uint32_t> &slab = dev->spillStack[dev->cur];
        const size_t words = needSpillSlab ? rt_stack_spill_bytes(imgW, imgH) / sizeof(uint32_t) : 0;
        if (words > slab.count) {
            dev->impure(); slab.reserve(words);
            void *flagDev = nullptr;
            HIP_CHECK(hipHostGetDevicePointer(&flagDev, dev->traversalOverflow, 0));
            HIP_CHECK(launch_stack_slab_init(slab.ptr, words / (RT_STACK_SPILL_HEADER + RT_STACK_SPILL), static_cast<const uint32_t *>(flagDev), dev->stream));
        }
        P.traversalStack = slab.ptr;
    }
    P.blueNoise = dev->blueNoise.ptr; P.counters = dev->counters.ptr;
    P.tileTiming = nullptr;
    if (dev->opt.tileTiming) { dev->tileTiming.reserve((size_t)RT_TIMING_WAVES * 2); P.tileTiming = dev->tileTiming.ptr; }
}

struct ImageInfo { const void *ptr; int srcBytes; int channels; int kind; };

static bool image_info(const ViewImages &I, int cur, int image, ImageInfo &info, size_t &dstPixelBytes) {
    switch (image) {
    case RT64_IMAGE_FINAL_RGBA8: info = { I.final, 4, 4, 0 }; dstPixelBytes = 4; return true;
    case RT64_IMAGE_SHADING_POSITION: info = { I.shadingPosition, 16, 4, 0 }; dstPixelBytes = 16; return true;
    case RT64_IMAGE_SHADING_NORMAL: info = { I.shadingNormal, 8, 4, 1 }; dstPixelBytes = 16; return true;
    case RT64_IMAGE_SHADING_SPECULAR: info = { I.shadingSpecular, 8, 4, 1 }; dstPixelBytes = 16; return true;
    case RT64_IMAGE_DIFFUSE: info = { I.diffuse, 4, 4, 2 }; dstPixelBytes = 16; return true;
    case RT64_IMAGE_INSTANCE_ID: info = { I.instanceId, 4, 1, 0 }; dstPixelBytes = 4; return true;
    case RT64_IMAGE_FIRST_INSTANCE_ID: info = { I.firstInstanceId, 4, 1, 0 }; dstPixelBytes = 4; return true;
    case RT64_IMAGE_DIRECT_LIGHT_RAW: info = { I.directLight[cur], 8, 4, 1 }; dstPixelBytes = 16; return true;
    case RT64_IMAGE_DIRECT_LIGHT_FILTERED: info = { I.filteredDirect[1], 8, 4, 1 }; dstPixelBytes = 16; return true;
    case RT64_IMAGE_INDIRECT_LIGHT_RAW: info = { I.indirectLight[cur], 8, 4, 1 }; dstPixelBytes = 16; return true;
    case RT64_IMAGE_INDIRECT_LIGHT_FILTERED: info = { I.filteredIndirect[1], 8, 4, 1 }; dstPixelBytes = 16; return true;
    case RT64_IMAGE_REFLECTION: info = { I.reflection, 8, 4, 1 }; dstPixelBytes = 16; return true;
    case RT64_IMAGE_REFRACTION: info = { I.refraction, 8, 4, 1 }; dstPixelBytes = 16; return true;
    case RT64_IMAGE_TRANSPARENT: info = { I.transparent, 8, 4, 1 }; dstPixelBytes = 16; return true;
    case RT64_IMAGE_VIEW_DIRECTION: info = { I.viewDirection, 8, 4, 1 }; dstPixelBytes = 16; return true;
    case RT64_IMAGE_FLOW: info = { I.flow, 4, 2, 1 }; dstPixelBytes = 8; return true;
    case RT64_IMAGE_REACTIVE_MASK: info = { I.reactiveMask, 1, 1, 2 }; dstPixelBytes = 4; return true;
    case RT64_IMAGE_LOCK_MASK: info = { I.lockMask, 1, 1, 2 }; dstPixelBytes = 4; return true;
    case RT64_IMAGE_DEPTH: info = { I.depth[cur], 4, 1, 0 }; dstPixelBytes = 4; return true;
    case RT64_IMAGE_OUTPUT_RGBA32F: info = { I.output, 16, 4, 0 }; dstPixelBytes = 16; return true;
    case RT64_IMAGE_PRIMARY_HIT: info = { I.primaryHit, 16, 4, 0 }; dstPixelBytes = 16; return true;
    case RT64_IMAGE_GI_MOMENTS: info = { I.moments[cur], 8, 2, 0 }; dstPixelBytes = 8; return true;
    case RT64_IMAGE_FILTER_GUIDE: info = { I.svgfGuide, 16, 4, 0 }; dstPixelBytes = 16; return true;
    case RT64_IMAGE_FILTER_PING: info = { I.filteredIndirect[0], 8, 4, 1 }; dstPixelBytes = 16; return true;
    default: return false;
    }
}

static void halo_exchange(Device *dev, const ViewImages &img, int W, int H, hipStream_t s);

void View::render() {
    Device *dev = scene->device;
    hipStream_t s = dev->stream;
    const bool prof = dev->profNow;
    const int slot = dev->cur;
    img.final = dev->finalOverride ? dev->finalOverride : finalBuf[slot];
    static const bool hostTiming = getenv("RT64_HOST_TIMING") != nullptr;
    auto hostPrev = std::chrono::steady_clock::now();
    auto mark = [&](int ev) {
        if (hostTiming) { auto now = std::chrono::steady_clock::now(); dev->hostStageUs[ev] += std::chrono::duration<double, std::micro>(now - hostPrev).count(); hostPrev = now; }
        if (prof) {
            if (dev->workSinceMark) { HIP_CHECK(hipEventRecord(dev->events[ev], s)); dev->eventAlias[ev] = ev; }
            else dev->eventAlias[ev] = dev->eventAlias[dev->lastMark];
            dev->lastMark = ev; dev->workSinceMark = false;
        }
        if (hostTiming) { auto now = std::chrono::steady_clock::now(); dev->hostEventUs += std::chrono::duration<double, std::micro>(now - hostPrev).count(); hostPrev = now; }
    };
    auto L = [&](hipError_t e) { HIP_CHECK(e); dev->workSinceMark = true; };
    if (!perspectiveSet) throw std::runtime_error("RT64_DrawDevice: RT64_SetViewPerspective was never called (fov must be > 0).");
    const int debugMode = dev->opt.visualizationMode;
    if (debugMode == RT64_IMAGE_FLOW && dev->ownedRows() < dev->height) throw std::runtime_error("RT64_DrawDevice: visualization_mode 13 (flow) is not drawn on a partitioned device.");
    const bool leanNow = !rtInstances.empty() && dev->opt.leanFrames && !upscaleActive && !anyNonOpaque && !anyReflection && !anyRefraction && !anyFog && giSamples == 0 && motionBlurStrength <= 0.0f && dev->leanHoldoff == 0 && subFrames == 1 && debugMode == 0;
    if (leanFrame && !leanNow) materialise();
    if (subFrames > 1 && (upscaleActive || rtRect || separatePost())) throw std::runtime_error("RT64_DrawDevice: primary_spp > 1 is not combined with an upscaler, a resolution scale, motion blur or a viewport rectangle.");
    FrameParams P;
    fillParams(P);
    const int cur = rtSwap ? 1 : 0;
    const size_t n = (size_t)imgW * imgH;
    mark(Device::EV_BUILD);
    bool fgFolded = false;
    if (!rtInstances.empty()) {
        if (anyNonOpaque && !img.klistA) {
            const size_t slots = (size_t)(RT64_MAX_HIT_QUERIES + 1) * n;
            void *a = nullptr, *b = nullptr, *c = nullptr;
            HIP_CHECK(hipMalloc(&a, slots * sizeof(uint4))); allocations.push_back(a);
            HIP_CHECK(hipMalloc(&b, slots * sizeof(uint2))); allocations.push_back(b);
            HIP_CHECK(hipMalloc(&c, n * sizeof(uint32_t))); allocations.push_back(c);
            img.klistA = static_cast<uint4 *>(a); img.klistB = static_cast<uint2 *>(b); img.klistCount = static_cast<uint32_t *>(c);
        }
        if (!anyNonOpaque && giSamples > 0 && (!img.bounceRecords || bounceSamples < giSamples)) {
            void *a = nullptr;
            HIP_CHECK(hipMalloc(&a, (size_t)giSamples * n * 2 * sizeof(uint4))); allocations.push_back(a);
            img.bounceRecords = static_cast<uint4 *>(a); bounceSamples = giSamples;
            void *l = nullptr, *c = nullptr, *r = nullptr;
            const size_t tilesAll = (size_t)((imgW + 15) / 16) * (size_t)((imgH + 15) / 16);
            HIP_CHECK(hipMalloc(&l, (size_t)giSamples * (tilesAll + std::min<size_t>(tilesAll, RT_MAX_BOUNCE_GROUPS)) * 256 * 2 * sizeof(uint32_t))); allocations.push_back(l);
            HIP_CHECK(hipMalloc(&c, (size_t)RT_MAX_BOUNCE_GROUPS * 2 * sizeof(uint32_t))); allocations.push_back(c);
            HIP_CHECK(hipMalloc(&r, (size_t)giSamples * n * sizeof(BounceRadiance))); allocations.push_back(r);
            img.bounceLists = static_cast<uint32_t *>(l); img.bounceCounts = static_cast<uint32_t *>(c); img.bounceResults = static_cast<BounceRadiance *>(r);
        }
        const bool klist = anyNonOpaque;
        reflStatePending = false;
        if (anyReflection && dev->opt.maxReflections > 0) {
            if (!img.reflState0) {
                void *a = nullptr, *b = nullptr, *c = nullptr;
                HIP_CHECK(hipMalloc(&a, n * sizeof(uint4))); allocations.push_back(a);
                HIP_CHECK(hipMalloc(&b, n * sizeof(uint4))); allocations.push_back(b);
                HIP_CHECK(hipMalloc(&c, n * sizeof(uint32_t))); allocations.push_back(c);
                HIP_CHECK(hipMemsetAsync(c, 0, n * sizeof(uint32_t), s));
                img.reflState0 = static_cast<uint4 *>(a); img.reflState1 = static_cast<uint4 *>(b); img.reflTag = static_cast<uint32_t *>(c);
            }
            reflStatePending = true; reflStateTag = P.frameCount + 1u; reflStateY0 = P.tileY0; reflStateY1 = P.tileY1;
        }
        const bool denoiseGI = denoiserEnabled && giSamples > 0;
        bool guideByResolve = false, inputByResolve = false;
        FrameParams X = P;
        bool haloExchange = false;
        if (denoiseGI && !P.separatePost && (P.tileY0 > 0 || P.tileY1 < imgH || P.stripCount > 1)) {
            if (P.stripCount > 1) throw std::runtime_error("RT64_DrawDevice: a frame with GI + denoiser filters across rows; partition it into contiguous bands (RT64_SetDeviceTile), not interleaved strips.");
            haloExchange = dev->opt.denoiserMode == 1 && dev->haloActive();
            const int halo = haloExchange ? std::max(dev->opt.haloMargin, SVGF_INPUT_HALO_ROWS) : (dev->opt.denoiserMode == 1 ? SVGF_HALO_ROWS : GAUSSIAN_HALO_ROWS);
            X.tileY0 = std::max(0, P.tileY0 - halo); X.tileY1 = std::min(imgH, P.tileY1 + halo);
        }
        const bool lean = leanNow;
        const bool fused = lean && dev->opt.fusedLean;
        const bool fusedFull = !lean && !klist && dev->opt.fusedLean && debugMode == 0;
        leanFrame = lean; fusedFrame = fused; fusedFullFrame = fusedFull; lastParams = P; lastCur = cur;
        if (!(fused && !P.separatePost && !rtRect && !dev->opt.leanRecords)) dev->impure();
        if (fused && !P.separatePost && !rtRect && rasterFgScreen.ready && rasterFgScreen.triTotal > 0 && dev->opt.foldForeground) {
            P.rasterFg = rasterFgScreen.table.ptr; P.rasterFgTris = rasterFgScreen.tris.ptr; P.rasterFgCount = rasterFgScreen.triTotal;
            fgFolded = true;
        }
        packedFinal = false;
        if (fused && !P.separatePost && !rtRect && (fgFolded || !(rasterFgScreen.ready && rasterFgScreen.triTotal > 0)) && dev->gatherTarget &&
            dev->gatherTargetBytes >= (size_t)dev->ownedRows() * (size_t)imgW * 4) {
            P.finalPacked = static_cast<uint32_t *>(dev->gatherTarget);
            packedFinal = true;
        }
        auto orderTiles = [&](FrameParams &F) -> unsigned {
            if (!(dev->opt.tileOrder && !F.cacheWords)) return 0u;
            const unsigned tiles = owned_tiles(F);
            if (tiles == 0u) return 0u;
            if (tileOrderTiles != tiles) {
                dev->impure();
                for (int k = 0; k < dev->streamCount; k++) {
                    tileCost[k].reserve(tiles); tileOrder[k].reserve(tiles);
                    HIP_CHECK(hipMemsetAsync(tileCost[k].ptr, 0, (size_t)tiles * 4, s));
                    tileOrderValid[k] = false;
                }
                tileOrderTiles = tiles;
            }
            F.tileCost = tileCost[slot].ptr; F.tileOrder = tileOrderValid[slot] ? tileOrder[slot].ptr : nullptr;
            return tiles;
        };
        const bool reflectBeside = anyReflection && dev->opt.maxReflections > 0 && denoiseGI && dev->opt.denoiserMode == 1 && dev->opt.overlapReflection;
        auto reflectOnAux = [&]() {
            if (!dev->auxStream) {
                HIP_CHECK(hipStreamCreateWithFlags(&dev->auxStream, hipStreamNonBlocking));
                HIP_CHECK(hipEventCreateWithFlags(&dev->forkEvent, hipEventDisableTiming)); HIP_CHECK(hipEventCreateWithFlags(&dev->joinEvent, hipEventDisableTiming));
            }
            HIP_CHECK(hipEventRecord(dev->forkEvent, s));
            HIP_CHECK(hipStreamWaitEvent(dev->auxStream, dev->forkEvent, 0));
            if (prof) { HIP_CHECK(hipEventRecord(dev->auxEvents[dev->evSet][0], dev->auxStream)); dev->auxTimed[dev->evSet] = true; }
            for (int r = 0; r < dev->opt.maxReflections; r++) L(launch_reflection(P, img, klist, r, r == dev->opt.maxReflections - 1, cur, dev->auxStream));
            if (prof) HIP_CHECK(hipEventRecord(dev->auxEvents[dev->evSet][1], dev->auxStream));
            HIP_CHECK(hipEventRecord(dev->joinEvent, dev->auxStream));
        };
        const bool reflectEarly = reflectBeside && !klist && !needSpillSlab;
        if (fused) {
            if (P.tileTiming) { HIP_CHECK(hipMemsetAsync(dev->tileTiming.ptr, 0, dev->tileTiming.bytes(), s)); }
            const unsigned ordered = orderTiles(P);
            L(launch_lean_frame(P, img, dev->opt.leanRecords ? hitInstance.ptr : nullptr, cur, false, 0, imgH, dev->opt.maxFrameGroups, s));
            if (ordered) { L(launch_tile_order(tileCost[slot].ptr, tileOrder[slot].ptr, ordered, s)); tileOrderValid[slot] = true; }
            fusedStoreless = !dev->opt.leanRecords;
            mark(Device::EV_PRIMARY_TRACE); mark(Device::EV_PRIMARY); mark(Device::EV_DIRECT);
        }
        else if (fusedFull) {
            if (P.stripCount > 1 && (X.tileY0 != P.tileY0 || X.tileY1 != P.tileY1)) throw std::runtime_error("RT64_DrawDevice: interleaved strips with a denoiser halo.");
            if (X.tileTiming) { HIP_CHECK(hipMemsetAsync(dev->tileTiming.ptr, 0, dev->tileTiming.bytes(), s)); }
            const unsigned ordered = orderTiles(X);
            L(launch_lean_frame(X, img, hitInstance.ptr, cur, true, P.tileY0, P.tileY1, dev->opt.maxFrameGroups, s));
            if (ordered) { L(launch_tile_order(tileCost[slot].ptr, tileOrder[slot].ptr, ordered, s)); tileOrderValid[slot] = true; }
            mark(Device::EV_PRIMARY_TRACE); mark(Device::EV_PRIMARY); mark(Device::EV_DIRECT);
            if (reflectEarly) reflectOnAux();
        }
        else {
            L(launch_primary_trace(X, img, hitInstance.ptr, klist, s));
            mark(Device::EV_PRIMARY_TRACE);
            L(launch_primary_shade(X, img, hitInstance.ptr, cur, anyNonOpaque, lean, s));
            mark(Device::EV_PRIMARY);
            L(launch_direct(P, img, cur, lean, s));
            mark(Device::EV_DIRECT);
            if (reflectEarly) reflectOnAux();
        }
        if (lean) {}
        else if (giSamples == 0) L(launch_indirect_constant(P, img, cur, s));
        else {
            bool refill = dev->opt.bounceRefill == 1;
            if (dev->opt.bounceRefill < 0) { size_t tri = 0; for (auto &ri : rtInstances) tri += ri.instance->mesh->blasCount; refill = tri >= 65536; }
            const bool split = dev->opt.bounceSplit == 1 || (dev->opt.bounceSplit < 0 && X.cacheWords != 0 && giSamples >= 2);
            const int walk = refill ? BOUNCE_WALK_REFILL : (split ? BOUNCE_WALK_SPLIT : BOUNCE_WALK_PLAIN);
            const unsigned groups = dev->opt.bounceGroups >= 0 ? (unsigned)dev->opt.bounceGroups : (walk == BOUNCE_WALK_PLAIN ? 1024u : 0u);
            guideByResolve = denoiseGI && dev->opt.denoiserMode == 1 && !klist && img.bounceRecords != nullptr && dev->opt.foldGuide;
            L(launch_indirect(X, img, cur, !denoiseGI, klist, walk, groups, guideByResolve ? (dev->opt.foldVariance ? 3 : 1) : 0, s));
            inputByResolve = guideByResolve && dev->opt.foldVariance;
// ... 649 lines not shown

}

using namespace rt64;

#define RT64_TRY try {
#define RT64_CATCH(ret) } catch (const std::exception &e) { GlobalLastError = e.what(); fprintf(stderr, "%s\n", e.what()); return ret; }
#define RT64_CATCH_VOID } catch (const std::exception &e) { GlobalLastError = e.what(); fprintf(stderr, "%s\n", e.what()); }

RT64_EXPORT const char *RT64_GetLastError() { return GlobalLastError.c_str(); }

static int env_int(const char *name, int def) { const char *e = getenv(name); return e && *e ? atoi(e) : def; }

RT64_EXPORT RT64_DEVICE *RT64_CreateDeviceHeadless(int width, int height, int hipDevice) {
    RT64_TRY return reinterpret_cast<RT64_DEVICE *>(new Device(width, height, hipDevice)); RT64_CATCH(nullptr)
}
RT64_EXPORT RT64_DEVICE *RT64_CreateDevice(void *hwnd) {
    (void)hwnd;
    return RT64_CreateDeviceHeadless(env_int("RT64_WIDTH", 1280), env_int("RT64_HEIGHT", 720), env_int("RT64_HIP_DEVICE", -1));
}
RT64_EXPORT void RT64_DestroyDevice(RT64_DEVICE *device) { RT64_TRY delete reinterpret_cast<Device *>(device); RT64_CATCH_VOID }
RT64_EXPORT void RT64_DrawDevice(RT64_DEVICE *device, int vsyncInterval, float deltaTimeMs) {
    RT64_TRY if (!device) throw std::runtime_error("RT64_DrawDevice: NULL device."); reinterpret_cast<Device *>(device)->draw(vsyncInterval, deltaTimeMs); RT64_CATCH_VOID
}
RT64_EXPORT void RT64_SetDeviceSize(RT64_DEVICE *device, int width, int height) {
    Device *d = reinterpret_cast<Device *>(device); if (d && width > 0 && height > 0) { d->pendingWidth = width; d->pendingHeight = height; }
}
RT64_EXPORT void RT64_SetDeviceTile(RT64_DEVICE *device, int y0, int y1) {
    Device *d = reinterpret_cast<Device *>(device); if (!d) return;
    if (y0 < 0 || y1 <= y0) { d->tileSet = false; d->tileY0 = 0; d->tileY1 = d->height; } else { d->tileSet = true; d->tileY0 = y0; d->tileY1 = y1; }
}
RT64_EXPORT void RT64_SetDeviceInterleave(RT64_DEVICE *device, int rank, int count) {
    Device *d = reinterpret_cast<Device *>(device); if (!d) return;
    if (count <= 1 || rank < 0 || rank >= count) { d->stripRank = 0; d->stripCount = 1; } else { d->stripRank = rank; d->stripCount = count; }
}
RT64_EXPORT size_t RT64_ReadbackDevice(RT64_DEVICE *device, int image, void *dst, size_t dstBytes) {
    RT64_TRY if (!device || !dst) throw std::runtime_error("RT64_ReadbackDevice: NULL argument."); return readback(reinterpret_cast<Device *>(device), image, dst, dstBytes, false); RT64_CATCH(0)
}
RT64_EXPORT size_t RT64_CopyDeviceImage(RT64_DEVICE *device, int image, void *devicePtr, size_t dstBytes) {
    RT64_TRY if (!device || !devicePtr) throw std::runtime_error("RT64_CopyDeviceImage: NULL argument."); return readback(reinterpret_cast<Device *>(device), image, devicePtr, dstBytes, true); RT64_CATCH(0)
}
RT64_EXPORT void RT64_SetDeviceGatherTarget(RT64_DEVICE *device, void *devicePtr, size_t bytes) {
    Device *d = reinterpret_cast<Device *>(device);
    if (!d) return;
    d->gatherTarget = devicePtr; d->gatherTargetBytes = devicePtr ? bytes : 0;
}
RT64_EXPORT int RT64_GetDeviceStats(RT64_DEVICE *device, RT64_FRAME_STATS *stats) {
    Device *d = reinterpret_cast<Device *>(device);
    if (!d || !stats || stats->structSize < 5 * sizeof(unsigned int)) return 0;
    d->use(); d->finishStats();
    RT64_FRAME_STATS full = d->stats; full.structSize = sizeof(RT64_FRAME_STATS);
    if (full.width == 0) { full.width = full.screenWidth = (unsigned)d->width; full.height = full.screenHeight = (unsigned)d->height; full.tileY0 = (unsigned)d->tileY0; full.tileY1 = (unsigned)d->tileY1; }
    const unsigned int n = stats->structSize < sizeof(RT64_FRAME_STATS) ? stats->structSize : (unsigned int)sizeof(RT64_FRAME_STATS);
    memcpy(stats, &full, n); stats->structSize = n;
    return 1;
}
RT64_EXPORT int RT64_SetDeviceOption(RT64_DEVICE *device, const char *key, double value) {
    Device *d = reinterpret_cast<Device *>(device); if (!d || !key) return 0;
    std::string k = key;
    if (k == "count_traversal") d->opt.countTraversal = value != 0.0;
    else if (k == "profile_passes") d->opt.profilePasses = value != 0.0;
    else if (k == "profile_every") { d->finishStats(); d->opt.profileEvery = std::max(1, (int)value); d->profCounter = 0; }
    else if (k == "sync_present") d->opt.syncPresent = value != 0.0;
    else if (k == "denoiser_mode") d->opt.denoiserMode = (int)value;
    else if (k == "bounce_refill") d->opt.bounceRefill = (int)value;
    else if (k == "overlap_reflection") d->opt.overlapReflection = value != 0.0;
    else if (k == "overlap_frames") d->opt.overlapFrames = value != 0.0;
    else if (k == "tile_order") d->opt.tileOrder = value != 0.0;
    else if (k == "fold_variance") d->opt.foldVariance = value != 0.0;
    else if (k == "fold_guide") d->opt.foldGuide = value != 0.0;
    else if (k == "fold_compose") d->opt.foldCompose = value != 0.0;
    else if (k == "halo_exchange") d->opt.haloExchange = value != 0.0;
    else if (k == "halo_dry_run") d->opt.haloDryRun = value != 0.0;
    else if (k == "halo_margin") d->opt.haloMargin = std::max((int)value, SVGF_INPUT_HALO_ROWS);
    else if (k == "bounce_split") d->opt.bounceSplit = (int)value;
    else if (k == "bounce_groups") d->opt.bounceGroups = value >= 0.0 && value <= (double)RT_MAX_BOUNCE_GROUPS ? (int)value : -1;
    else if (k == "tile_timing") d->opt.tileTiming = value != 0.0;
    else if (k == "lds_cache") d->opt.ldsCache = value != 0.0;
    else if (k == "lean_records") d->opt.leanRecords = value != 0.0;
    else if (k == "host_tlas") d->opt.hostTlas = value != 0.0;
    else if (k == "frame_prologue") d->opt.framePrologue = value != 0.0;
    else if (k == "simple_kernels") d->opt.simpleKernels = value != 0.0;
    else if (k == "reset_accum") { d->finishStats(); d->accum = RT64_FRAME_STATS(); }
    else if (k == "fold_foreground") d->opt.foldForeground = value != 0.0;
    else if (k == "fused_lean") d->opt.fusedLean = value != 0.0;
    else if (k == "lean_frames") d->opt.leanFrames = value != 0.0;
    else if (k == "always_rebuild") d->opt.alwaysRebuild = value != 0.0;
    else if (k == "max_reflections") d->opt.maxReflections = std::max(0, (int)value);
    else if (k == "motion_blur_samples") { if (!(value >= 0.0 && value <= 1024.0) || value != std::floor(value)) return 0; d->opt.motionBlurSamples = (uint32_t)value; }
    else if (k == "visualization_mode") { if (!(value >= 0.0 && value <= 16.0) || value != std::floor(value)) return 0; d->opt.visualizationMode = (int)value; }
    else if (k == "generate_mipmaps") { if (value != 0.0 && value != 1.0) return 0; d->opt.generateMipmaps = value != 0.0; }
    else if (k == "gi_bounces") { if (value != 1.0 && value != 2.0) return 0; d->opt.giBounces = (int)value; }
    else if (k == "primary_spp") { if (!(value >= 1.0 && value <= 64.0)) return 0; d->opt.primarySpp = (int)value; }
    else if (k == "max_frame_groups") d->opt.maxFrameGroups = value >= 1.0 && value <= (double)RT_MAX_FRAME_GROUPS ? (unsigned)value : RT_MAX_FRAME_GROUPS;
    else return 0;
    return 1;
}
RT64_EXPORT size_t RT64_ReadbackTileTiming(RT64_DEVICE *device, void *dst, size_t dstBytes) {
    RT64_TRY
    Device *d = reinterpret_cast<Device *>(device);
    if (!d || !dst || !d->tileTiming.ptr) throw std::runtime_error("RT64_ReadbackTileTiming: set the device option tile_timing and draw a frame first.");
    d->enter();
    const size_t bytes = std::min(dstBytes, d->tileTiming.bytes());
    HIP_CHECK(hipMemcpyAsync(dst, d->tileTiming.ptr, bytes, hipMemcpyDeviceToHost, d->stream));
    HIP_CHECK(hipStreamSynchronize(d->stream));
    return bytes;
    RT64_CATCH(0)
}
RT64_EXPORT void *RT64_GetDeviceStream(RT64_DEVICE *device) { Device *d = reinterpret_cast<Device *>(device); return d ? d->stream : nullptr; }

RT64_EXPORT RT64_VIEW *RT64_CreateView(RT64_SCENE *scenePtr) {
    RT64_TRY if (!scenePtr) throw std::runtime_error("RT64_CreateView: NULL scene."); return reinterpret_cast<RT64_VIEW *>(new View(reinterpret_cast<Scene *>(scenePtr))); RT64_CATCH(nullptr)
}
RT64_EXPORT void RT64_SetViewPerspective(RT64_VIEW *viewPtr, RT64_MATRIX4 viewMatrix, float fovRadians, float nearDist, float farDist, bool canReproject) {
    View *v = reinterpret_cast<View *>(viewPtr); if (!v) return;
    v->view = mat_from(viewMatrix); v->fov = fovRadians; v->nearDist = nearDist; v->farDist = farDist; v->canReproject = canReproject; v->perspectiveSet = fovRadians > 0.0f;
}
RT64_EXPORT void RT64_SetViewDescription(RT64_VIEW *viewPtr, RT64_VIEW_DESC viewDesc) {
    View *v = reinterpret_cast<View *>(viewPtr); if (!v) return;
    v->resolutionScale = viewDesc.resolutionScale; v->motionBlurStrength = viewDesc.motionBlurStrength; v->maxLights = viewDesc.maxLights;
    v->diSamples = viewDesc.diSamples; v->giSamples = viewDesc.giSamples; v->denoiserEnabled = viewDesc.denoiserEnabled;
    v->upscaler = viewDesc.upscaler; v->upscalerMode = viewDesc.upscalerMode; v->upscalerSharpness = viewDesc.upscalerSharpness;
}
RT64_EXPORT void RT64_SetViewSkyPlane(RT64_VIEW *viewPtr, RT64_TEXTURE *texturePtr) { View *v = reinterpret_cast<View *>(viewPtr); if (v) v->skyPlane = reinterpret_cast<Texture *>(texturePtr); }
RT64_EXPORT RT64_INSTANCE *RT64_GetViewRaytracedInstanceAt(RT64_VIEW *viewPtr, int x, int y) {
    RT64_TRY
    View *v = reinterpret_cast<View *>(viewPtr); if (!v) return nullptr;
    Device *dev = v->scene->device; dev->enter();
    const float xs = (float)v->imgW / (float)dev->width, ys = (float)v->imgH / (float)dev->height;
    x = (int)lroundf(x * xs); y = (int)lroundf(y * ys);
    if (x < 0 || x >= v->imgW || y < 0 || y >= v->imgH) return nullptr;
    int32_t id = -1;
    v->materialise();
    HIP_CHECK(hipMemcpyAsync(&id, v->img.firstInstanceId + (size_t)y * v->imgW + x, 4, hipMemcpyDeviceToHost, dev->stream));
    HIP_CHECK(hipStreamSynchronize(dev->stream));
    if (id >= 0 && (size_t)id < v->rtInstances.size()) return reinterpret_cast<RT64_INSTANCE *>(v->rtInstances[id].instance);
    return nullptr;
    RT64_CATCH(nullptr)
}
RT64_EXPORT int RT64_TraceViewRays(RT64_VIEW *view, const RT64_RAY *rays, RT64_RAY_HIT *hits, size_t count, unsigned int flags) {
    RT64_TRY run_view_query("RT64_TraceViewRays", reinterpret_cast<View *>(view), rays, hits, nullptr, count, flags, nullptr, true, QUERY_TRACE); return 1; RT64_CATCH(0)
}
RT64_EXPORT int RT64_TraceViewRaysDevice(RT64_VIEW *view, const void *rays, void *hits, size_t count, unsigned int flags, void *stream) {
    RT64_TRY run_view_query("RT64_TraceViewRaysDevice", reinterpret_cast<View *>(view), rays, hits, nullptr, count, flags, stream, false, QUERY_TRACE); return 1; RT64_CATCH(0)
}
RT64_EXPORT int RT64_ResolveViewRayHits(RT64_VIEW *view, const RT64_RAY *rays, const RT64_RAY_HIT *hits, RT64_RAY_SURFACE *surfaces, size_t count) {
    RT64_TRY run_view_query("RT64_ResolveViewRayHits", reinterpret_cast<View *>(view), rays, const_cast<RT64_RAY_HIT *>(hits), surfaces, count, 0, nullptr, true, QUERY_RESOLVE); return 1; RT64_CATCH(0)
}
RT64_EXPORT int RT64_ResolveViewRayHitsDevice(RT64_VIEW *view, const void *rays, const void *hits, void *surfaces, size_t count, void *stream) {
    RT64_TRY run_view_query("RT64_ResolveViewRayHitsDevice", reinterpret_cast<View *>(view), rays, const_cast<void *>(hits), surfaces, count, 0, stream, false, QUERY_RESOLVE); return 1; RT64_CATCH(0)
}
RT64_EXPORT int RT64_ShadeViewRayHits(RT64_VIEW *view, const RT64_RAY *rays, const RT64_RAY_HIT *hits, const float *lods, RT64_RAY_MATERIAL *materials, size_t count) {
    RT64_TRY run_view_query("RT64_ShadeViewRayHits", reinterpret_cast<View *>(view), rays, const_cast<RT64_RAY_HIT *>(hits), materials, count, 0, nullptr, true, QUERY_SHADE, lods); return 1; RT64_CATCH(0)
}
RT64_EXPORT int RT64_ShadeViewRayHitsDevice(RT64_VIEW *view, const void *rays, const void *hits, const void *lods, void *materials, size_t count, void *stream) {
    RT64_TRY run_view_query("RT64_ShadeViewRayHitsDevice", reinterpret_cast<View *>(view), rays, const_cast<void *>(hits), materials, count, 0, stream, false, QUERY_SHADE, lods); return 1; RT64_CATCH(0)
}
RT64_EXPORT int RT64_TraceViewRayMaterials(RT64_VIEW *view, const RT64_RAY *rays, RT64_RAY_HIT *hits, const float *lods, RT64_RAY_MATERIAL *materials, size_t count, unsigned int flags) {
    RT64_TRY run_view_query("RT64_TraceViewRayMaterials", reinterpret_cast<View *>(view), rays, hits, materials, count, flags, nullptr, true, QUERY_TRACE | QUERY_SHADE, lods); return 1; RT64_CATCH(0)
}
RT64_EXPORT int RT64_TraceViewRaySurfaces(RT64_VIEW *view, const RT64_RAY *rays, RT64_RAY_HIT *hits, RT64_RAY_SURFACE *surfaces, size_t count, unsigned int flags) {
    RT64_TRY run_view_query("RT64_TraceViewRaySurfaces", reinterpret_cast<View *>(view), rays, hits, surfaces, count, flags, nullptr, true, QUERY_TRACE | QUERY_RESOLVE); return 1; RT64_CATCH(0)
}
RT64_EXPORT int RT64_TraceViewRaysAlpha(RT64_VIEW *view, const RT64_RAY *rays, const float *lods, RT64_RAY_HIT *hits, size_t count, unsigned int flags) {
    RT64_TRY run_view_query("RT64_TraceViewRaysAlpha", reinterpret_cast<View *>(view), rays, hits, nullptr, count, flags, nullptr, true, QUERY_ALPHA, lods); return 1; RT64_CATCH(0)
}
// ... 714 lines not shown
```

### sm64rt-legacy-renderer_amd/csrc/trace.h

```cpp
#pragma once
#include "kernels.h"
#include "device_math.h"

typedef const FrameParams __attribute__((address_space(4))) &PRef;
typedef const FrameParams __attribute__((address_space(4))) *PPtr;
struct Mat16c { float m[16]; };
DEV Mat16c cmat(const float __attribute__((address_space(4))) *p) { Mat16c r; __builtin_memcpy(&r, p, sizeof(r)); return r; }
typedef const ViewImages __attribute__((address_space(4))) &IRef;
typedef const ViewImages __attribute__((address_space(4))) *IPtr;
#define RT_KERNARG_IMAGES_OFFSET ((sizeof(FrameParams) + alignof(ViewImages) - 1) / alignof(ViewImages) * alignof(ViewImages))
DEV IPtr kernel_images() { return (IPtr)((const char __attribute__((address_space(4))) *)__builtin_amdgcn_kernarg_segment_ptr() + RT_KERNARG_IMAGES_OFFSET); }
DEV IPtr kernel_images_here() { uint32_t z; asm volatile("s_mov_b32 %0, 0" : "=s"(z)); return (IPtr)((const char __attribute__((address_space(4))) *)__builtin_amdgcn_kernarg_segment_ptr() + RT_KERNARG_IMAGES_OFFSET + z); }
DEV PPtr kernel_params() { return (PPtr)__builtin_amdgcn_kernarg_segment_ptr(); }
DEV PPtr kernel_params_here() { uint32_t z; asm volatile("s_mov_b32 %0, 0" : "=s"(z)); return (PPtr)((const char __attribute__((address_space(4))) *)__builtin_amdgcn_kernarg_segment_ptr() + z); }
#define RT_BLOCK 256
#define RT_LANES 64

struct RaySpace { float o[3], d[3], inv[3], oi[3]; };

DEV void make_ray_space(const float o[3], const float d[3], RaySpace &r) {
#pragma unroll
    for (int k = 0; k < 3; k++) {
        r.o[k] = o[k]; r.d[k] = d[k];
        float ds = fabsf(d[k]) < 1e-20f ? copysignf(1e-20f, d[k]) : d[k];
// ... 10 lines not shown
    float tf = fminf(fminf(fmaxf(ax, bx), fmaxf(ay, by)), fminf(fmaxf(az, bz), tmax)) * 1.0000004f;
    tnear = tn;
    return tn <= tf;
}

DEV bool tri_hit(const RaySpace &r, const GpuTri &tri, bool cull, float tmin, float tmax, float &t, float &u, float &v) {
    float e1[3], e2[3], p[3], q[3], tv[3];
#pragma unroll
    for (int k = 0; k < 3; k++) { e1[k] = tri.v1[k] - tri.v0[k]; e2[k] = tri.v2[k] - tri.v0[k]; }
    g_cross3(r.d, e2, p);
    float det = g_dot3(e1, p);
    const bool detRejected = cull ? !(det > 0.0f) : (det == 0.0f || det != det);
    float inv = 1.0f / det;
#pragma unroll
    for (int k = 0; k < 3; k++) tv[k] = r.o[k] - tri.v0[k];
    float uu = g_dot3(tv, p) * inv;
    g_cross3(tv, e1, q);
    float vv = g_dot3(r.d, q) * inv;
    float tt = g_dot3(e2, q) * inv;
    if (detRejected || !(uu >= 0.0f) || !(vv >= 0.0f) || !(uu + vv <= 1.0f) || !(tt > tmin) || !(tt < tmax)) return false;
    t = tt; u = uu; v = vv;
    return true;
}

typedef uint32_t u32x4_lds __attribute__((ext_vector_type(4)));

typedef uint32_t __attribute__((address_space(3))) *LdsU32Ptr;
typedef uint32_t __attribute__((address_space(1))) *GlobalU32Ptr;
typedef int16_t __attribute__((address_space(3))) *LdsI16Ptr;
#define RT_CACHE_INDEX_MASK 0x7FFFu
struct TraceStack {
    LdsU32Ptr lds;
    LdsI16Ptr lds16;
    GlobalU32Ptr spill;
    const u32x4_lds *cache;
    int ldsEntries;
    DEV void use_cache(const u32x4_lds *c) { cache = c; ldsEntries = RT_STACK_LDS_CACHED; }
    DEV void report_overflow() const {
        typedef uint32_t *__attribute__((address_space(1))) *FlagSlot;
        uint32_t *flag = *reinterpret_cast<FlagSlot>(reinterpret_cast<uintptr_t>(spill - RT_STACK_SPILL_HEADER));
        if (flag) __hip_atomic_fetch_add(flag, 1u, __ATOMIC_RELAXED, __HIP_MEMORY_SCOPE_SYSTEM);
    }
    template <bool LDS_ONLY = false> DEV void push(int &sp, uint32_t v) const {
        if (LDS_ONLY) { lds16[(sp & (RT_STACK_LDS_CACHED - 1)) * RT_LANES] = (int16_t)v; sp++; return; }
        if (sp < ldsEntries) lds[sp * RT_LANES] = v;
        else if (sp < ldsEntries + RT_STACK_SPILL) spill[sp - ldsEntries] = v;
        else { report_overflow(); return; }
        sp++;
    }
    template <bool LDS_ONLY = false> DEV uint32_t pop(int &sp) const {
        sp--;
        if (LDS_ONLY) return (uint32_t)(int32_t)lds16[(sp & (RT_STACK_LDS_CACHED - 1)) * RT_LANES];
        return sp < ldsEntries ? lds[sp * RT_LANES] : spill[sp - ldsEntries];
    }
};

struct TraceCounts { uint32_t nodes, tris; };

template <class T> DEV T load_global(const T *p) {
    typedef const T __attribute__((address_space(1))) *GP;
    return *reinterpret_cast<GP>(reinterpret_cast<uintptr_t>(p));
}
typedef uint32_t u32x4 __attribute__((ext_vector_type(4)));
typedef const u32x4 __attribute__((address_space(1))) *GlobalU4;
DEV GpuNode load_node(const GpuNode *p) {
    GlobalU4 q = reinterpret_cast<GlobalU4>(reinterpret_cast<uintptr_t>(p));
    union { u32x4 w[4]; GpuNode n; } u;
    u.w[0] = q[0]; u.w[1] = q[1]; u.w[2] = q[2]; u.w[3] = q[3];
    return u.n;
}
DEV GpuTri load_tri(const GpuTri *p) {
    GlobalU4 q = reinterpret_cast<GlobalU4>(reinterpret_cast<uintptr_t>(p));
    union { u32x4 w[3]; GpuTri t; } u;
    u.w[0] = q[0]; u.w[1] = q[1]; u.w[2] = q[2];
    return u.t;
}

DEV GpuNode load_node_lds(const u32x4_lds *q) {
    union { u32x4_lds w[4]; GpuNode n; } u;
    u.w[0] = q[0]; u.w[1] = q[1]; u.w[2] = q[2]; u.w[3] = q[3];
    return u.n;
}

DEV void fill_scene_cache(PRef P, u32x4_lds *cache) {
    constexpr uint32_t CHUNKS = RT_CACHE_MAX_WORDS / RT_BLOCK;
    static_assert(RT_CACHE_MAX_WORDS % RT_BLOCK == 0, "the scene cache is filled in chunks of RT_BLOCK words");
    GlobalU4 src = reinterpret_cast<GlobalU4>(reinterpret_cast<uintptr_t>(P.cacheImage));
    const uint32_t words = P.cacheWords;
    if (words != 0 && words <= (uint32_t)RT_CACHE_MAX_WORDS) {
        const uint32_t last = words - 1u;
        u32x4 w[CHUNKS];
#pragma unroll
        for (uint32_t k = 0; k < CHUNKS; k++) { const uint32_t t = threadIdx.x + k * RT_BLOCK; w[k] = src[t < last ? t : last]; }
#pragma unroll
        for (uint32_t k = 0; k < CHUNKS; k++) asm volatile("" : "+v"(w[k]));
#pragma unroll
        for (uint32_t k = 0; k < CHUNKS; k++) { const uint32_t t = threadIdx.x + k * RT_BLOCK; if (t < words) cache[t] = w[k]; }
    }
    __syncthreads();
}


union NodeOrTri { u32x4 w[4]; GpuNode n; GpuTri t; };
template <class OnHit>
DEV void trace_ray_stepwise(PRef P, const float o[3], const float d[3], float tmin, float tmax, bool cullBackFaces,
                            const TraceStack &stk, OnHit &&onHit, TraceCounts &cnt) {
    RaySpace W, R;
    make_ray_space(o, d, W);
    R = W;
    const GpuNode *nodes = P.tlasNodes;
    const GpuTri *tris = nullptr;
    int sp = 0, blasBase = -1;
    uint32_t inst = 0, instFlags = 0;
    float instDepthBias = 0.0f;
    bool cull = false;
    uint32_t cur = 0;
    bool alive = true;
    auto popNext = [&]() -> bool {
        if (blasBase >= 0 && sp == blasBase) { blasBase = -1; R = W; nodes = P.tlasNodes; }
        if (sp == 0) return false;
        cur = stk.pop(sp);
        return true;
    };
    while (alive) {
        const bool isNode = !(cur & RT64_LEAF_BIT), isTri = !isNode && cur != RT64_NO_CHILD && blasBase >= 0;
        NodeOrTri rec;
        if (isNode || isTri) {
            const uintptr_t at = isNode ? reinterpret_cast<uintptr_t>(nodes + cur) : reinterpret_cast<uintptr_t>(tris + (cur & 0x7FFFFFFFu));
            GlobalU4 q = reinterpret_cast<GlobalU4>(at);
            rec.w[0] = q[0]; rec.w[1] = q[1]; rec.w[2] = q[2]; rec.w[3] = q[3];
        }
        if (isNode) {
            cnt.nodes++;
            float tl, tr;
            const bool hl = box_hit(R, rec.n.lmin, rec.n.lmax, tmin, tmax, tl);
            const bool hr = box_hit(R, rec.n.rmin, rec.n.rmax, tmin, tmax, tr);
            const bool both = hl && hr, rightFirst = tr < tl;
            const uint32_t nearChild = both ? (rightFirst ? rec.n.right : rec.n.left) : (hl ? rec.n.left : rec.n.right);
            if (both) stk.push(sp, rightFirst ? rec.n.left : rec.n.right);
            if (hl || hr) cur = nearChild;
            else alive = popNext();
        }
        else if (isTri) {
            cnt.tris++;
            float t, u, v;
            if (tri_hit(R, rec.t, cull, tmin, tmax, t, u, v) && onHit(t, u, v, inst, rec.t.prim, tmax, instFlags, instDepthBias)) alive = false;
            else alive = popNext();
        }
        else if (cur != RT64_NO_CHILD) {
            inst = load_global(P.tlasIndex + (cur & 0x7FFFFFFFu));
            const GpuInstance *in = P.instances + inst;
            const float *M = in->worldToObject;
            float oo[3], dd[3];
#pragma unroll
            for (int c = 0; c < 3; c++) {
                const float m0 = load_global(M + c), m1 = load_global(M + 4 + c), m2 = load_global(M + 8 + c), m3 = load_global(M + 12 + c);
                oo[c] = fmaf(W.o[2], m2, fmaf(W.o[1], m1, fmaf(W.o[0], m0, m3)));
                dd[c] = fmaf(W.d[2], m2, fmaf(W.d[1], m1, W.d[0] * m0));
            }
            nodes = load_global(&in->nodes); tris = load_global(&in->tris);
            const uint32_t flags = load_global(&in->flags); instDepthBias = load_global(&in->material.depthBias);
            make_ray_space(oo, dd, R);
            instFlags = flags;
            cull = cullBackFaces && !(flags & GPU_INST_CULL_DISABLE);
            blasBase = sp;
            cur = 0;
        }
        else alive = popNext();
    }
}

template <bool CACHED = false, class OnHit>
// ... 173 lines not shown
```

Baseline: 19810.

## Skip primary tracing for tiles outside projected instance bounds

Projects the host-built TLAS instance boxes to screen space on the host and records, per tile row, the span of tiles that may hit geometry. Tiles outside the span skip the primary ray trace and are shaded as sky, and single-tile sky groups also skip committing the LDS scene cache fill. The span computation is cached keyed on camera and box data. It adds host work and kernel parameters, and relies on conservative margins to avoid missing geometry.

Result: faster. 20060, median of 6 (+1.3%).

```diff
diff --git a/sm64rt-legacy-renderer_amd/csrc/pass_common.h b/sm64rt-legacy-renderer_amd/csrc/pass_common.h
--- a/sm64rt-legacy-renderer_amd/csrc/pass_common.h
+++ b/sm64rt-legacy-renderer_amd/csrc/pass_common.h
@@ -31,6 +31,21 @@
     return tile_pixel_at<SHAPE>(P, tile, threadIdx.x >> 6, threadIdx.x & 63);
 }
 
+DEV bool sky_span_test(PRef P, uint32_t lt, uint32_t tx) {
+    const uint32_t row = lt * (uint32_t)P.stripCount + (uint32_t)P.stripRank;
+    const uint32_t at = row < (uint32_t)RT_SKY_SPAN_ROWS ? row : (uint32_t)RT_SKY_SPAN_ROWS - 1u;
+    const uint32_t span = *reinterpret_cast<const uint32_t __attribute__((address_space(4))) *>(&P.skySpans[at][0]);
+    return (row < P.skySpanRows) & ((tx < (span & 0xFFFFu)) | (tx >= (span >> 16)));
+}
+DEV bool sky_tile(PRef P, uint32_t tile) {
+    const uint32_t tilesX = ((uint32_t)P.width + 15u) >> 4;
+    return sky_span_test(P, tile / tilesX, tile % tilesX);
+}
+DEV bool sky_tile_by_reciprocal(PRef P, uint32_t tile, uint32_t reciprocal) {
+    const uint32_t tilesX = ((uint32_t)P.width + 15u) >> 4, lt = __umulhi(tile, reciprocal);
+    return sky_span_test(P, lt, tile - lt * tilesX);
+}
+
 DEV bool row_owned(PRef P, int y) { return (((y - P.tileY0) / 16) % P.stripCount) == P.stripRank; }
 
 constexpr uint32_t stack_words(bool cached) { return cached ? RT_STACK_LDS_CACHED / 2 : RT_STACK_LDS; }
@@ -57,11 +72,11 @@
     if (CACHED) env.stk.use_cache(dynLds);
 }
 template <bool CACHED, bool STATIC_COLUMNS = true, int BLOCK = RT_BLOCK>
-DEV void shading_env(PRef P, ShadeEnv &env, uint32_t *ldsStack, float *ldsLightIntensity, uint8_t *ldsLightIndex, u32x4_lds *dynLds) {
+DEV void shading_env(PRef P, ShadeEnv &env, uint32_t *ldsStack, float *ldsLightIntensity, uint8_t *ldsLightIndex, u32x4_lds *dynLds, bool fill = true) {
     env.stk = make_stack(P, ldsStack, stack_words(CACHED)); env.cnt = TraceCounts(); env.shadowRays = 0;
     if (STATIC_COLUMNS) light_columns(env, ldsLightIntensity, ldsLightIndex, RT64_MAX_LIGHTS + 1);
     if (STATIC_COLUMNS && !CACHED) return;
-    if (CACHED) { fill_scene_cache(P, dynLds); env.stk.use_cache(dynLds); }
+    if (CACHED) { if (fill) fill_scene_cache(P, dynLds); env.stk.use_cache(dynLds); }
     float *li = reinterpret_cast<float *>(dynLds + (CACHED ? P.cacheWords : 0u));
     light_columns(env, li, reinterpret_cast<uint8_t *>(li + light_slots(P) * (CACHED ? blockDim.x : (uint32_t)BLOCK)), light_slots(P));
 }
diff --git a/sm64rt-legacy-renderer_amd/csrc/passes.hip b/sm64rt-legacy-renderer_amd/csrc/passes.hip
--- a/sm64rt-legacy-renderer_amd/csrc/passes.hip
+++ b/sm64rt-legacy-renderer_amd/csrc/passes.hip
@@ -304,14 +304,20 @@
     return tileSeq < tiles;
 }
 template <bool CACHED, bool FULL, int WAVES, int BLOCK = RT_BLOCK>
-__global__ __launch_bounds__(BLOCK, WAVES) void lean_frame_kernel(FrameParams Pv, ViewImages Iv, int32_t *hitInstance, int cur, int ownedY0, int ownedY1) {
+__global__ __launch_bounds__(BLOCK, WAVES) void lean_frame_kernel(FrameParams Pv, ViewImages Iv, int32_t *hitInstance, int cur, int ownedY0, int ownedY1, uint32_t skyReciprocal) {
     PRef P = *kernel_params(); IRef I = *kernel_images(); (void)Pv; (void)Iv; (void)I;
     __shared__ uint32_t ldsStack[stack_words(CACHED) * BLOCK];
     extern __shared__ u32x4_lds dynLds[];
-    ShadeEnv env; shading_env<CACHED, false, BLOCK>(P, env, ldsStack, nullptr, nullptr, dynLds);
+    constexpr bool SPANS = BLOCK == RT_BLOCK && CACHED;
+    const bool oneTile = SPANS && skyReciprocal != 0u;
+    SceneCacheLoads cacheLoads;
+    if (CACHED) fill_scene_cache_issue(P, cacheLoads);
+    const bool skyGroup = oneTile && sky_tile_by_reciprocal(P, gridDim.x - 1u - blockIdx.x, skyReciprocal);
+    ShadeEnv env; shading_env<CACHED, false, BLOCK>(P, env, ldsStack, nullptr, nullptr, dynLds, false);
+    if (CACHED && !skyGroup) fill_scene_cache_commit(P, dynLds, cacheLoads);
+    const uint32_t tiles = tile_count(P);
     uint32_t rays = 0;
     TraceCounts primaryCnt = TraceCounts();
-    const uint32_t tiles = tile_count(P);
     const uint32_t trips = BLOCK == RT_BLOCK ? tiles : ((tiles + 7u) / 8u) * 32u;
     if (P.tileTiming && (threadIdx.x & 63u) == 0u) {
         uint32_t hwId; asm volatile("s_getreg_b32 %0, hwreg(HW_REG_HW_ID)" : "=s"(hwId));
@@ -331,7 +337,11 @@
     for (uint32_t trip = blockIdx.x; trip < trips; trip += gridDim.x) {
         PRef P = *kernel_params_here(); IRef I = *kernel_images_here();
         Pixel p;
-        if (BLOCK == RT_BLOCK) p = tile_pixel(P, tiles - 1u - trip);
+        bool sky = false;
+        if (BLOCK == RT_BLOCK) {
+            p = tile_pixel(P, tiles - 1u - trip);
+            sky = SPANS && (oneTile ? skyGroup : (P.skySpanRows != 0u && sky_tile(P, tiles - 1u - trip)));
+        }
         else {
             uint32_t tileSlot, quadrant;
             flush_cost(P);
@@ -348,7 +358,9 @@
         RayDiff noDiff; noDiff.dOdx = noDiff.dOdy = noDiff.dDdx = noDiff.dDdy = mk3s(0.0f);
         SurfaceHit h;
         const TraceCounts before = env.cnt;
-        const uint32_t nhits = trace_surface<false, CACHED>(P, env, I, i, o, rayDirection, noDiff, px, py, h);
+        uint32_t nhits = 0;
+        if (sky) { h.hit = false; h.key = INFINITY; h.t = h.u = h.v = 0.0f; h.instance = h.prim = 0u; }
+        else nhits = trace_surface<false, CACHED>(P, env, I, i, o, rayDirection, noDiff, px, py, h);
         primaryCnt.nodes += env.cnt.nodes - before.nodes; primaryCnt.tris += env.cnt.tris - before.tris;
         rays++;
         const bool keepRecords = FULL || hitInstance != nullptr;
@@ -1125,9 +1137,11 @@
         grid = (grid + 31u) / 32u * 32u;
         lds = lds / (RT_BLOCK / 64) + 16;
     }
+    const unsigned tilesX = (unsigned)(P.width + 15) / 16u;
+    const uint32_t skyReciprocal = (P.cacheWords && P.skySpanRows && grid == tiles && tilesX >= 2u && tilesX < 4096u) ? (uint32_t)(0x100000000ull / tilesX) + 1u : 0u;
     return with_flag(P.cacheWords != 0, [&](auto CACHED) { return with_flag(full, [&](auto FULL) {
         constexpr int BLOCK = decltype(CACHED)::value ? RT_BLOCK : 64;
-        return launch(lean_frame_kernel<decltype(CACHED)::value, decltype(FULL)::value, LEAN_WAVES, BLOCK>, grid, BLOCK, lds, s, P, I, hitInstance, cur, ownedY0, ownedY1);
+        return launch(lean_frame_kernel<decltype(CACHED)::value, decltype(FULL)::value, LEAN_WAVES, BLOCK>, grid, BLOCK, lds, s, P, I, hitInstance, cur, ownedY0, ownedY1, skyReciprocal);
     }); });
 }
 hipError_t RT_LAUNCHER(launch_indirect)(const FrameParams &P, const ViewImages &I, int cur, bool writeFiltered, bool klist, int walk, unsigned groups, int writeGuide, hipStream_t s) {
diff --git a/sm64rt-legacy-renderer_amd/csrc/rt64_gpu.h b/sm64rt-legacy-renderer_amd/csrc/rt64_gpu.h
--- a/sm64rt-legacy-renderer_amd/csrc/rt64_gpu.h
+++ b/sm64rt-legacy-renderer_amd/csrc/rt64_gpu.h
@@ -1,6 +1,7 @@
 #pragma once
 #include <stdint.h>
 #include "../../include/rt64.h"
+#include "tile_coverage.h"
 
 #define RT64_LEAF_BIT 0x80000000u
 #define RT64_NO_CHILD 0xFFFFFFFFu
@@ -107,7 +108,9 @@
     uint32_t simpleKernels;
     uint32_t separatePost;
     const float *postSource; int32_t postSourceW, postSourceH;
-    const GpuRasterInstance *rasterFg; const void *rasterFgTris; uint32_t rasterFgCount, rasterFgPad;
+    const GpuRasterInstance *rasterFg; const void *rasterFgTris; uint32_t rasterFgCount;
+    uint32_t skySpanRows;
+    uint16_t skySpans[RT_SKY_SPAN_ROWS][2];
     uint32_t *finalPacked;
     float skyBase[4];
     const uint32_t *skyTiled; uint32_t skyTiledLog2W, skyTiledLog2H;
diff --git a/sm64rt-legacy-renderer_amd/csrc/rt64_host.cpp b/sm64rt-legacy-renderer_amd/csrc/rt64_host.cpp
--- a/sm64rt-legacy-renderer_amd/csrc/rt64_host.cpp
+++ b/sm64rt-legacy-renderer_amd/csrc/rt64_host.cpp
@@ -126,6 +126,7 @@
 struct Options {
     bool countTraversal = false, profilePasses = true, syncPresent = true, alwaysRebuild = false, leanFrames = true, fusedLean = true, foldForeground = true;
     int profileEvery = 1;
+    bool skySpans = true;
     bool leanRecords = false;
     bool framePrologue = true;
     bool hostTlas = true;
@@ -371,6 +372,7 @@
         std::vector<uint8_t> uploadedTables;
         DevArray<uint8_t> cacheImage; bool cacheImageValid = false;
         const uint8_t *cacheImageAt = nullptr; std::vector<uint64_t> cacheBlasKey;
+        std::vector<float> boxLo, boxHi;
         unsigned readers = 0;
         std::vector<hipEvent_t> queryEvents;
     } tab[TABLE_SLOTS];
@@ -385,6 +387,8 @@
     bool fusedStoreless = false;
     bool fusedFrame = false;
     FrameParams lastParams; int lastCur = 0;
+    struct SkySpanCache { enum { KEY_WORDS = 38 + 6 * 64 }; uint32_t key[KEY_WORDS]; size_t keyWords = 0; uint32_t rows = 0; uint16_t spans[RT_SKY_SPAN_ROWS][2]; } skySpanCache[2];
+    void skySpans(FrameParams &F, int which);
     struct QueryScene {
         bool valid = false;
         bool meshDestroyed = false;
@@ -978,8 +982,8 @@
 static inline float gmin(float a, float b) { return (a < b || (a == b && std::signbit(a))) ? a : b; }
 static inline float gmax(float a, float b) { return (a > b || (a == b && !std::signbit(a))) ? a : b; }
 static void host_build_tlas(const GpuInstance *inst, const float (*meshMin)[3], const float (*meshMax)[3], uint32_t n,
-                            GpuNode *nodes, uint32_t *sortedIndex, uint32_t *morton, BlasHeader *header) {
-    std::vector<float> lo(3 * (size_t)n), hi(3 * (size_t)n);
+                            GpuNode *nodes, uint32_t *sortedIndex, uint32_t *morton, BlasHeader *header, std::vector<float> &lo, std::vector<float> &hi) {
+    lo.resize(3 * (size_t)n); hi.resize(3 * (size_t)n);
     float smin[3] = { INFINITY, INFINITY, INFINITY }, smax[3] = { -INFINITY, -INFINITY, -INFINITY };
     for (uint32_t i = 0; i < n; i++) {
         float bmn[3] = { INFINITY, INFINITY, INFINITY }, bmx[3] = { -INFINITY, -INFINITY, -INFINITY };
@@ -1181,6 +1185,7 @@
         if (pick < 0) { pick = (tabCur + 1) % TABLE_SLOTS; dev->impure(); }
         tabCur = pick;
         tab[tabCur].readers = 0;
+        tab[tabCur].boxLo.clear(); tab[tabCur].boxHi.clear();
         for (hipEvent_t ev : tab[tabCur].queryEvents) HIP_CHECK(hipStreamWaitEvent(dev->stream, ev, 0));
         const uint32_t n = (uint32_t)nInst;
         const bool hostTlas = n >= 1 && n <= RT64_HOST_TLAS_MAX && dev->opt.hostTlas;
@@ -1205,7 +1210,7 @@
                 uint32_t *hi = reinterpret_cast<uint32_t *>(hh + 1), *hm = hi + n;
                 float mn[RT64_HOST_TLAS_MAX][3], mx[RT64_HOST_TLAS_MAX][3];
                 for (uint32_t i = 0; i < n; i++) { memcpy(mn[i], rtInstances[i].instance->mesh->hostBmin, 12); memcpy(mx[i], rtInstances[i].instance->mesh->hostBmax, 12); }
-                host_build_tlas(hInst, mn, mx, n, hn, hi, hm, hh);
+                host_build_tlas(hInst, mn, mx, n, hn, hi, hm, hh, tab[tabCur].boxLo, tab[tabCur].boxHi);
                 if (hostCache) {
                     memset(pinnedStage + tlasAt + nodeBytes + sizeof(BlasHeader) + 2 * sizeof(uint32_t) * n, 0, cacheAt - (tlasAt + nodeBytes + sizeof(BlasHeader) + 2 * sizeof(uint32_t) * n));
                     uint32_t *cw = reinterpret_cast<uint32_t *>(pinnedStage + cacheAt);
@@ -1347,7 +1352,7 @@
     P.separatePost = separatePost() ? 1u : 0u;
     P.simpleKernels = simpleFrame ? 1u : 0u;
     P.postSource = img.output; P.postSourceW = imgW; P.postSourceH = imgH;
-    P.rasterFg = nullptr; P.rasterFgTris = nullptr; P.rasterFgCount = 0; P.rasterFgPad = 0; P.finalPacked = nullptr;
+    P.rasterFg = nullptr; P.rasterFgTris = nullptr; P.rasterFgCount = 0; P.finalPacked = nullptr;
     memset(&P.background, 0, sizeof(P.background));
     if (rasterBgEnv.ready) { P.background.texels = background.ptr; P.background.width = (uint32_t)backgroundW; P.background.height = (uint32_t)backgroundH; P.background.mips = 1; P.background.pow2 = ((backgroundW & (backgroundW - 1)) == 0 && (backgroundH & (backgroundH - 1)) == 0) ? 1u : 0u; }
     if (P.separatePost) { P.tileY0 = 0; P.tileY1 = imgH; P.stripRank = 0; P.stripCount = 1; }
@@ -1388,6 +1393,28 @@
     P.blueNoise = dev->blueNoise.ptr; P.counters = dev->counters.ptr;
     P.tileTiming = nullptr;
     if (dev->opt.tileTiming) { dev->tileTiming.reserve((size_t)RT_TIMING_WAVES * 2); P.tileTiming = dev->tileTiming.ptr; }
+    skySpans(P, 0);
+}
+
+void View::skySpans(FrameParams &F, int which) {
+    Device *dev = scene->device;
+    const TableSlot &T = tab[tabCur];
+    F.skySpanRows = 0;
+    if (!dev->opt.skySpans || dev->opt.countTraversal || !F.cacheWords || T.boxLo.empty()) return;
+    SkySpanCache &C = skySpanCache[which];
+    const size_t nBox = T.boxLo.size(), keyWords = 38 + 2 * nBox;
+    static_assert(SkySpanCache::KEY_WORDS == 38 + 6 * RT64_HOST_TLAS_MAX, "the span cache key holds the boxes of a host-built TLAS");
+    uint32_t key[SkySpanCache::KEY_WORDS];
+    if (keyWords > (size_t)SkySpanCache::KEY_WORDS) return;
+    memcpy(&key[0], F.viewI, 64); memcpy(&key[16], F.projectionI, 64); memcpy(&key[32], F.pixelJitter, 8);
+    key[34] = (uint32_t)F.width; key[35] = (uint32_t)F.height; key[36] = (uint32_t)F.tileY0; key[37] = (uint32_t)F.tileY1;
+    memcpy(&key[38], T.boxLo.data(), 4 * nBox); memcpy(&key[38 + nBox], T.boxHi.data(), 4 * nBox);
+    if (keyWords != C.keyWords || memcmp(key, C.key, 4 * keyWords) != 0) {
+        C.rows = tile_coverage_spans(F.viewI, F.projectionI, F.pixelJitter, F.width, F.height, F.tileY0, F.tileY1, T.boxLo.data(), T.boxHi.data(), (uint32_t)(nBox / 3), C.spans, RT_SKY_SPAN_ROWS);
+        memcpy(C.key, key, 4 * keyWords); C.keyWords = keyWords;
+    }
+    F.skySpanRows = C.rows;
+    if (C.rows) memcpy(F.skySpans, C.spans, sizeof(C.spans[0]) * C.rows);
 }
 
 struct ImageInfo { const void *ptr; int srcBytes; int channels; int kind; };
@@ -1496,6 +1523,7 @@
             haloExchange = dev->opt.denoiserMode == 1 && dev->haloActive();
             const int halo = haloExchange ? std::max(dev->opt.haloMargin, SVGF_INPUT_HALO_ROWS) : (dev->opt.denoiserMode == 1 ? SVGF_HALO_ROWS : GAUSSIAN_HALO_ROWS);
             X.tileY0 = std::max(0, P.tileY0 - halo); X.tileY1 = std::min(imgH, P.tileY1 + halo);
+            skySpans(X, 1);
         }
         const bool lean = leanNow;
         const bool fused = lean && dev->opt.fusedLean;
@@ -2311,6 +2339,7 @@
     else if (k == "frame_prologue") d->opt.framePrologue = value != 0.0;
     else if (k == "simple_kernels") d->opt.simpleKernels = value != 0.0;
     else if (k == "reset_accum") { d->finishStats(); d->accum = RT64_FRAME_STATS(); }
+    else if (k == "sky_spans") d->opt.skySpans = value != 0.0;
     else if (k == "fold_foreground") d->opt.foldForeground = value != 0.0;
     else if (k == "fused_lean") d->opt.fusedLean = value != 0.0;
     else if (k == "lean_frames") d->opt.leanFrames = value != 0.0;
diff --git a/sm64rt-legacy-renderer_amd/csrc/tile_coverage.h b/sm64rt-legacy-renderer_amd/csrc/tile_coverage.h
--- /dev/null
+++ b/sm64rt-legacy-renderer_amd/csrc/tile_coverage.h
@@ -0,0 +1,91 @@
+#pragma once
+#include <stdint.h>
+#include <math.h>
+
+#define RT_SKY_SPAN_ROWS 256
+
+struct TileCoverageRule {
+    bool clip = true;
+    double slackUlps = 16.0;
+    double marginPixels = 1.0;
+    double clipT = 0.05;
+};
+
+static inline uint32_t tile_coverage_spans(const float *viewI, const float *projectionI, const float *pixelJitter, int width, int height, int tileY0, int tileY1,
+                                           const float *lo, const float *hi, uint32_t boxes, uint16_t (*spans)[2], uint32_t maxRows,
+                                           const TileCoverageRule &rule = TileCoverageRule()) {
+    if (width <= 0 || height <= 0 || tileY1 <= tileY0 || tileY0 < 0 || width > 16 * 65535) return 0;
+    const uint32_t rows = (uint32_t)(tileY1 - tileY0 + 15) / 16u;
+    if (rows > maxRows) return 0;
+    const double jx = pixelJitter[0], jy = pixelJitter[1], jmax = fmax(fabs(jx), fabs(jy));
+    if (!(jmax <= 1.0)) return 0;
+    double a[3][3];
+    for (int k = 0; k < 3; k++) {
+        double c0 = 0.0, c1 = 0.0, c2 = 0.0;
+        for (int j = 0; j < 3; j++) {
+            const double v = viewI[4 * j + k];
+            c0 += (double)projectionI[j] * v; c1 -= (double)projectionI[4 + j] * v; c2 += ((double)projectionI[8 + j] + (double)projectionI[12 + j]) * v;
+        }
+        a[0][k] = c0; a[1][k] = c1; a[2][k] = c2;
+    }
+    const double eye[3] = { viewI[12], viewI[13], viewI[14] };
+    auto cross = [](const double *u, const double *v, double *r) { r[0] = u[1] * v[2] - u[2] * v[1]; r[1] = u[2] * v[0] - u[0] * v[2]; r[2] = u[0] * v[1] - u[1] * v[0]; };
+    auto dot = [](const double *u, const double *v) { return u[0] * v[0] + u[1] * v[1] + u[2] * v[2]; };
+    double inv[3][3];
+    cross(a[1], a[2], inv[0]); cross(a[2], a[0], inv[1]); cross(a[0], a[1], inv[2]);
+    const double det = dot(a[0], inv[0]);
+    const double scale = sqrt(dot(a[0], a[0]) * dot(a[1], a[1]) * dot(a[2], a[2]));
+    if (!isfinite(det) || !isfinite(scale) || !(fabs(det) > 1e-12 * scale)) return 0;
+    for (int r = 0; r < 3; r++) for (int k = 0; k < 3; k++) inv[r][k] /= det;
+    for (int k = 0; k < 3; k++) if (!isfinite(eye[k])) return 0;
+
+    const uint32_t tilesX = (uint32_t)(width + 15) / 16u;
+    for (uint32_t r = 0; r < rows; r++) { spans[r][0] = 0; spans[r][1] = 0; }
+    const double margin = rule.marginPixels + jmax;
+    for (uint32_t b = 0; b < boxes; b++) {
+        double mag = fmax(fabs(eye[0]), fmax(fabs(eye[1]), fabs(eye[2])));
+        for (int k = 0; k < 3; k++) { if (!isfinite(lo[3 * b + k]) || !isfinite(hi[3 * b + k])) return 0; mag = fmax(mag, fmax(fabs((double)lo[3 * b + k]), fabs((double)hi[3 * b + k]))); }
+        const double slack = rule.slackUlps * ldexp(mag, -23);
+        double glo[3], ghi[3];
+        bool inside = true, empty = false;
+        for (int k = 0; k < 3; k++) {
+            glo[k] = (double)lo[3 * b + k] - slack; ghi[k] = (double)hi[3 * b + k] + slack;
+            if (lo[3 * b + k] > hi[3 * b + k]) empty = true;
+            if (!(eye[k] >= glo[k] && eye[k] <= ghi[k])) inside = false;
+        }
+        if (empty || inside) return 0;
+        double q[8][3];
+        for (int c = 0; c < 8; c++) {
+            const double p[3] = { ((c & 1) ? ghi[0] : glo[0]) - eye[0], ((c & 2) ? ghi[1] : glo[1]) - eye[1], ((c & 4) ? ghi[2] : glo[2]) - eye[2] };
+            for (int r = 0; r < 3; r++) q[c][r] = dot(inv[r], p);
+        }
+        double u0 = INFINITY, u1 = -INFINITY, v0 = INFINITY, v1 = -INFINITY;
+        bool any = false, bad = false;
+        auto take = [&](double x, double y, double z) {
+            const double u = (x / z + 1.0) * 0.5 * (double)width - 0.5, v = (y / z + 1.0) * 0.5 * (double)height - 0.5;
+            if (!isfinite(u) || !isfinite(v)) { bad = true; return; }
+            u0 = fmin(u0, u); u1 = fmax(u1, u); v0 = fmin(v0, v); v1 = fmax(v1, v); any = true;
+        };
+        for (int c = 0; c < 8; c++) if (q[c][2] >= rule.clipT) take(q[c][0], q[c][1], q[c][2]);
+        if (rule.clip) for (int c = 0; c < 8; c++) for (int axis = 1; axis < 8; axis <<= 1) {
+            if (c & axis) continue;
+            const double *p0 = q[c], *p1 = q[c | axis];
+            if ((p0[2] >= rule.clipT) == (p1[2] >= rule.clipT)) continue;
+            const double s = (rule.clipT - p0[2]) / (p1[2] - p0[2]);
+            take(p0[0] + s * (p1[0] - p0[0]), p0[1] + s * (p1[1] - p0[1]), rule.clipT);
+        }
+        if (bad) return 0;
+        if (!any) continue;
+        u0 -= margin; u1 += margin; v0 -= margin; v1 += margin;
+        if (u1 < 0.0 || u0 > (double)(width - 1) || v1 < (double)tileY0 || v0 > (double)(tileY1 - 1)) continue;
+        const double tx0 = floor(u0 / 16.0), tx1 = floor(u1 / 16.0) + 1.0, ty0 = floor((v0 - (double)tileY0) / 16.0), ty1 = floor((v1 - (double)tileY0) / 16.0);
+        const uint32_t x0 = tx0 < 0.0 ? 0u : (uint32_t)tx0, x1 = tx1 > (double)tilesX ? tilesX : (uint32_t)tx1;
+        const uint32_t r0 = ty0 < 0.0 ? 0u : (uint32_t)ty0, r1 = ty1 > (double)(rows - 1) ? rows - 1 : (uint32_t)ty1;
+        if (x0 >= x1) continue;
+        for (uint32_t r = r0; r <= r1; r++) {
+            if (spans[r][0] == spans[r][1]) { spans[r][0] = (uint16_t)x0; spans[r][1] = (uint16_t)x1; }
+            else { if (x0 < spans[r][0]) spans[r][0] = (uint16_t)x0; if (x1 > spans[r][1]) spans[r][1] = (uint16_t)x1; }
+        }
+    }
+    return rows;
+}
diff --git a/sm64rt-legacy-renderer_amd/csrc/trace.h b/sm64rt-legacy-renderer_amd/csrc/trace.h
--- a/sm64rt-legacy-renderer_amd/csrc/trace.h
+++ b/sm64rt-legacy-renderer_amd/csrc/trace.h
@@ -116,12 +116,35 @@
     return u.n;
 }
 
-DEV void fill_scene_cache(PRef P, u32x4_lds *cache) {
-    constexpr uint32_t CHUNKS = RT_CACHE_MAX_WORDS / RT_BLOCK;
-    static_assert(RT_CACHE_MAX_WORDS % RT_BLOCK == 0, "the scene cache is filled in chunks of RT_BLOCK words");
+constexpr uint32_t RT_CACHE_CHUNKS = RT_CACHE_MAX_WORDS / RT_BLOCK;
+static_assert(RT_CACHE_MAX_WORDS % RT_BLOCK == 0, "the scene cache is filled in chunks of RT_BLOCK words");
+struct SceneCacheLoads { u32x4 w[RT_CACHE_CHUNKS]; };
+DEV bool scene_cache_words_ok(uint32_t words) { return words != 0 && words <= (uint32_t)RT_CACHE_MAX_WORDS; }
+DEV void fill_scene_cache_issue(PRef P, SceneCacheLoads &f) {
     GlobalU4 src = reinterpret_cast<GlobalU4>(reinterpret_cast<uintptr_t>(P.cacheImage));
     const uint32_t words = P.cacheWords;
-    if (words != 0 && words <= (uint32_t)RT_CACHE_MAX_WORDS) {
+    if (scene_cache_words_ok(words)) {
+        const uint32_t last = words - 1u;
+#pragma unroll
+        for (uint32_t k = 0; k < RT_CACHE_CHUNKS; k++) { const uint32_t t = threadIdx.x + k * RT_BLOCK; f.w[k] = src[t < last ? t : last]; }
+    }
+    asm volatile("" ::: "memory");
+}
+DEV void fill_scene_cache_commit(PRef P, u32x4_lds *cache, SceneCacheLoads &f) {
+    const uint32_t words = P.cacheWords;
+    if (scene_cache_words_ok(words)) {
+#pragma unroll
+        for (uint32_t k = 0; k < RT_CACHE_CHUNKS; k++) asm volatile("" : "+v"(f.w[k]));
+#pragma unroll
+        for (uint32_t k = 0; k < RT_CACHE_CHUNKS; k++) { const uint32_t t = threadIdx.x + k * RT_BLOCK; if (t < words) cache[t] = f.w[k]; }
+    }
+    __syncthreads();
+}
+DEV void fill_scene_cache(PRef P, u32x4_lds *cache) {
+    constexpr uint32_t CHUNKS = RT_CACHE_CHUNKS;
+    GlobalU4 src = reinterpret_cast<GlobalU4>(reinterpret_cast<uintptr_t>(P.cacheImage));
+    const uint32_t words = P.cacheWords;
+    if (scene_cache_words_ok(words)) {
         const uint32_t last = words - 1u;
         u32x4 w[CHUNKS];
 #pragma unroll
```
